# jhorstmann/queryengine

Measured on AMD Instinct MI355X. Metric: rows/sec filter+project over int64/f64 batch; achieved HBM GB/s in roofline, higher is better.
Workload: dtype int64/f64

## Files before the change

### include/qe_hip.h

```cpp
#ifndef QE_HIP_H
#define QE_HIP_H

#include <stddef.h>
#include <stdint.h>

#ifdef __cplusplus
extern "C" {
#endif

#define QE_ABI_VERSION 1

enum {
    QE_OK = 0,
    QE_ERR_INVALID_ARG = 1,
    QE_ERR_PROGRAM = 2,
    QE_ERR_HIP = 3,
    QE_ERR_OOM = 4,
    QE_ERR_UNSUPPORTED = 5,
    QE_ERR_INTERNAL = 6,
    QE_ERR_COMM = 7
};

enum {
    QE_STRING = 0,
// ... 175 lines not shown
int32_t qe_result_order_by_keys(qe_ctx *ctx, const qe_result *result, const qe_sort_key *keys, int32_t nkeys, int64_t limit,
                                qe_result **out);
int32_t qe_ctx_last_sort_stats(const qe_ctx *ctx, int64_t out[4]);

enum { QE_JOIN_INNER = 0, QE_JOIN_LEFT = 1, QE_JOIN_SEMI = 2, QE_JOIN_ANTI = 3 };
typedef struct { const qe_result *result; const qe_batch *batch; } qe_join_input;
typedef struct qe_join_table qe_join_table;

int32_t qe_join_build(qe_ctx *ctx, const qe_join_input *build, const int32_t *key_cols, int32_t nkeys,
                      qe_join_table **out);
int64_t qe_join_table_rows(const qe_join_table *table);
void    qe_join_table_free(qe_ctx *ctx, qe_join_table *table);
int32_t qe_join_probe(qe_ctx *ctx, const qe_join_table *table, const qe_join_input *probe,
                      const int32_t *key_cols, int32_t nkeys, int32_t join_type,
                      const int32_t *probe_out_cols, int32_t nprobe_out,
                      const int32_t *build_out_cols, int32_t nbuild_out, qe_result **out);
int32_t qe_ctx_last_join_stats(const qe_ctx *ctx, int64_t out[4]);

enum { QE_WIN_ROW_NUMBER = 0, QE_WIN_RANK, QE_WIN_DENSE_RANK,
       QE_WIN_SUM, QE_WIN_COUNT, QE_WIN_MIN, QE_WIN_MAX, QE_WIN_AVG,
       QE_WIN_LAG, QE_WIN_LEAD };
typedef struct { int32_t fn; int32_t column; int64_t offset; } qe_window_fn;
int32_t qe_result_window(qe_ctx *ctx, const qe_result *result,
                         const int32_t *partition_cols, int32_t npart,
                         const qe_sort_key *order, int32_t norder,
                         const qe_window_fn *fns, int32_t nfn, qe_result **out);
#define QE_FRAME_UNBOUNDED (-1)
enum { QE_WIN_FIRST_VALUE = 10, QE_WIN_LAST_VALUE = 11 };
typedef struct { int32_t fn; int32_t column; int64_t offset;
                 int64_t preceding; int64_t following; } qe_window_frame_fn;
int32_t qe_result_window_frames(qe_ctx *ctx, const qe_result *result,
                                const int32_t *partition_cols, int32_t npart,
                                const qe_sort_key *order, int32_t norder,
                                const qe_window_frame_fn *fns, int32_t nfn, qe_result **out);
int32_t qe_ctx_last_window_stats(const qe_ctx *ctx, int64_t out[4]);

enum { QE_OSA_COUNT_DISTINCT = 0, QE_OSA_PERCENTILE_CONT = 1, QE_OSA_PERCENTILE_DISC = 2, QE_OSA_MODE = 3 };
typedef struct { int32_t fn; int32_t column; double fraction; } qe_ordered_agg;
int32_t qe_result_group_ordered(qe_ctx *ctx, const qe_result *result,
                                const int32_t *group_cols, int32_t ngroup,
                                const qe_ordered_agg *fns, int32_t nfn, qe_result **out);
int32_t qe_ctx_last_ordered_stats(const qe_ctx *ctx, int64_t out[4]);

enum { QE_SET_UNION = 0, QE_SET_INTERSECT = 1, QE_SET_EXCEPT = 2 };
int32_t qe_result_set_op(qe_ctx *ctx, const qe_result *left, const qe_result *right,
                         int32_t op, int32_t all, qe_result **out);
int32_t qe_ctx_last_set_stats(const qe_ctx *ctx, int64_t out[4]);

enum { QE_ASOF_BACKWARD = 0, QE_ASOF_FORWARD = 1 };
int32_t qe_result_asof_join(qe_ctx *ctx, const qe_result *left, const qe_result *right,
                            const int32_t *left_by, const int32_t *right_by, int32_t nby,
                            int32_t left_on, int32_t right_on,
                            int32_t direction, int32_t strict, int32_t join_type,
                            const int32_t *left_out, int32_t nleft_out,
                            const int32_t *right_out, int32_t nright_out, qe_result **out);
int32_t qe_ctx_last_asof_stats(const qe_ctx *ctx, int64_t out[4]);

int32_t qe_batch_from_result(qe_ctx *ctx, const qe_result *result, qe_batch **out);

typedef struct { char internal[128]; } qe_comm_id;
int32_t qe_comm_unique_id(qe_ctx *ctx, qe_comm_id *out);
int32_t qe_comm_init(qe_ctx *ctx, int32_t nranks, int32_t rank, const qe_comm_id *id);
int32_t qe_comm_rank(const qe_ctx *ctx);
int32_t qe_comm_nranks(const qe_ctx *ctx);
void qe_comm_destroy(qe_ctx *ctx);
int32_t qe_gather(qe_ctx *ctx, const qe_result *local, int32_t root, qe_result **out);
int32_t qe_filter_project_gather(qe_ctx *ctx, const qe_batch *batch, const qe_expr *filter, const qe_expr *const *projections,
                                 int32_t nproj, int32_t root, int32_t nslices, qe_result **out);
int32_t qe_comm_allgather_host(qe_ctx *ctx, const void *send, size_t nbytes, void *recv);

int32_t qe_filter_project_source(qe_ctx *ctx, const qe_batch *batch, const qe_expr *filter,
                                 const qe_expr *const *projections, int32_t nproj, const char **out);
int32_t qe_filter_project_geometry(qe_ctx *ctx, const qe_batch *batch, const qe_expr *filter,
                                   const qe_expr *const *projections, int32_t nproj, int32_t *out_chosen,
                                   int32_t *out_from_cache);
int32_t qe_filter_project_conjunct_order(qe_ctx *ctx, const qe_batch *batch, const qe_expr *filter,
                                         const qe_expr *const *projections, int32_t nproj, int32_t *out_order, int32_t capacity,
                                         int32_t *out_nconj);
enum { QE_FORM_RING = 0, QE_FORM_TWO_PASS = 1, QE_FORM_DENSE = 2, QE_FORM_PER_NODE = 3, QE_FORM_NO_FILTER = 4,
       QE_FORM_LOCAL = 5 ,
        QE_FORM_GROUPBY_DENSE = 8, QE_FORM_GROUPBY_HASHED = 9,
       QE_FORM_GROUPBY_HASH_PARTITIONED = 10  };
int32_t qe_ctx_last_form(const qe_ctx *ctx);
int32_t qe_stream_read_bandwidth(qe_ctx *ctx, int64_t nbytes, int32_t reps, double *out_gbps);

int32_t qe_stream_read_write_time(qe_ctx *ctx, int64_t nbytes, int32_t write_every, int32_t reps, double *out_ms,
                                  double *out_written_bytes);

#ifdef __cplusplus
}
#endif
#endif
```

### queryengine_amd/csrc/qe_api.cpp

```cpp
#include <algorithm>
#include <cmath>
#include <cstdio>
#include <cstdlib>
#include <functional>
#include <sstream>

#include "qe_exec.h"
#include "qe_kernels.h"
#include "qe_pernode.h"
#include "qe_scan.h"

using namespace qe;

namespace {

constexpr double kDenseFromSelectivity = 0.12;
constexpr double kLocalUpToSelectivity = 0.03;
constexpr int64_t kSampleFromRows = 8ll << 20;

FusedGeometry geometry_of(const qe_ctx *ctx) {
    FusedGeometry g;
    const int t = ctx->opts.tuning[0], u = ctx->opts.tuning[1];
    if (t == 64 || t == 128 || t == 256 || t == 512 || t == 1024) g.threads = t;
    const int mw = ctx->opts.tuning[3] / 100;
// ... 139 lines not shown
    plan->kernel = ctx->jit->get(plan->cg.source, "qe_fused", rq.load);
    ctx->plans[k] = plan;
    return plan;
}

}

namespace {

void PlanGeometry::narrow_plan_wide_candidate() {
    if (wide && !in.dense && !agg_fns && in.group_keys.empty()) {
        size_t inbytes = 0;
        for (int c : plan->cg.used_cols) inbytes += (size_t)value_bytes(in.schema[(size_t)c].type);
        if (inbytes <= 16) {
            const FusedGeometry dflt = geometry_of(ctx);
            in.geo.subs_per_chunk = dflt.subs_per_chunk;
            in.geo.ring_entries = dflt.ring_entries;
        }
    }
}

void PlanGeometry::lds_table_1024_threads() {
    if (!in.group_keys.empty() && !plan->cg.hashed && !plan->cg.table_in_lds && ctx->opts.tuning[0] == 0 &&
        (size_t)plan->cg.ngroups * plan->cg.table_words * 8 <= 144 * 1024) {
        in.geo.threads = 1024;
        analyze();
    }
}

void PlanGeometry::hash_partitioned_tile() {
    if (plan->cg.hp && ctx->opts.tuning[1] == 0 && ctx->opts.tuning[0] == 0) {
        in.geo.threads = 512;
        int u = 4;
        auto lines_lds = [&](int uu) {
            const size_t R = (size_t)std::max(1, plan->cg.hp_line_recs), P = (size_t)plan->cg.nparts;
            const size_t tile = (size_t)(in.geo.threads / 64) * 128 * uu, lines = (tile + (P <= 256 ? 2 : 1) * (R - 1) * P + R - 1) / R;
            return lines * 132 + ((P + 3) & ~(size_t)3) * (P <= 256 ? 24 : 16) + 64;
        };
        if (plan->cg.hp_line_recs && lines_lds(4) > 156 * 1024) {
            in.hp_lines = 0;
            analyze();
        }
        if (plan->cg.hp_line_recs) {
            while (u > 1 && lines_lds(u) > 156 * 1024) u /= 2;
        } else {
            const size_t rec = (size_t)(1 + plan->cg.nvals) * 8;
            while (u > 1 && (size_t)(in.geo.threads / 64) * 128 * u * rec > 128 * 1024) u /= 2;
        }
        in.geo.unroll = u;
    }
}

void PlanGeometry::partitioned_tile_512_threads() {
    if (plan->cg.partitioned && !plan->cg.hp && plan->cg.nparts > 128 && ctx->opts.tuning[0] == 0 && in.geo.threads == 256 &&
        8 + plan->cg.part_shift + 13 <= 32 && (size_t)8 * in.geo.sub_rows() * (1 + plan->cg.nvals) * 8 <= 128 * 1024) {
        in.geo.threads = 512;
    }
}

void PlanGeometry::hashed_unroll() {
    if (plan->cg.hashed && ctx->opts.tuning[1] == 0 && in.geo.unroll > 4) {
        in.geo.unroll = 4;
    }
}

void PlanGeometry::dense_lds_tile() {
    if (in.dense) {
        const size_t rowbytes = std::max<size_t>(output_row_bytes(plan->cg.outs), 1);
        auto tile_bytes = [&]() { return (size_t)(in.geo.threads / 64) * 128 * in.geo.unroll * rowbytes; };
        const size_t limit = 64 * 1024;
        while (tile_bytes() > limit && in.geo.unroll > 1 && ctx->opts.tuning[1] == 0) in.geo.unroll /= 2;
        while (tile_bytes() > limit && in.geo.threads > 128 && ctx->opts.tuning[0] == 0) in.geo.threads /= 2;
        if (tile_bytes() > 150 * 1024)
            fail(QE_ERR_UNSUPPORTED, "projection list too wide for the dense kernel's LDS tile (" + std::to_string(rowbytes) + " bytes per output row)");
    }
}

void PlanGeometry::ring_lds_budget() {
    if (!agg_fns && in.filter && !in.dense) {
        const size_t rowbytes = std::max<size_t>(output_row_bytes(plan->cg.outs), 1);
        if (ctx->opts.tuning[7] / 100 == 0) in.geo.nbuf = 2;
        if (ctx->opts.tuning[0] == 0) {
            const size_t limit = 96 * 1024;
            while (in.geo.threads > 64 && (size_t)(in.geo.threads / 64) * in.geo.nbuf * in.geo.ring_entries * rowbytes > limit)
                in.geo.threads /= 2;
        }
        if ((size_t)(in.geo.threads / 64) * in.geo.nbuf * in.geo.ring_entries * rowbytes > 156 * 1024)
            fail(QE_ERR_UNSUPPORTED, "projection list too wide for the fused kernel's LDS buffers (" + std::to_string(rowbytes) +
                                         " bytes per output row); use QE_EXEC_PER_NODE");
    }
}

void PlanGeometry::register_estimate() {
    auto dwords = [](int t) { return (t == QE_DOUBLE || t == QE_INT64) ? 2 : 1; };
    for (;;) {
        int in_dw = 0, out_dw = 0, nbool = 1, in_nulls = 0;
        for (int c : plan->cg.used_cols) {
            in_dw += dwords(in.schema[c].type);
            in_nulls += in.schema[c].nullable ? 1 : 0;
        }
        for (const OutSpec &o : plan->cg.outs) {
            out_dw += dwords(o.type);
            nbool += o.nullable ? 1 : 0;
        }
        const int est = 2 * in.geo.unroll * (std::max(in_dw, out_dw) + nbool - 1) + (in_nulls ? in.geo.unroll : 0) + 54;
        plan->est_regs = est;
        if (((est > 168 && in.geo.unroll > 4) || (est > 300 && in.geo.unroll > 2)) && ctx->opts.tuning[1] == 0 && !wide) {
            in.geo.unroll /= 2;
            if (!in.dense) in.geo.subs_per_chunk *= 2;
            continue;
        }
        in.geo.min_waves = est <= 120 ? 4 : est <= 168 ? 3 : est <= 256 ? 2 : 1;
        break;
    }
}

void PlanGeometry::compile_without_scratch() {
    for (;;) {
        plan->cg = generate_fused_source(in);
        plan->kernel = ctx->jit->get(plan->cg.source, "qe_fused", false);
        if (ctx->jit->last_scratch <= 0) break;
        const bool can_retry = in.geo.min_waves > 1 || (in.geo.unroll > 2 && ctx->opts.tuning[1] == 0);
        if (can_retry) ctx->jit->reject(plan->cg.source, ctx->jit->last_scratch);
        if (in.geo.min_waves > 2) {
            in.geo.min_waves--;
        } else if (in.geo.unroll > 2 && ctx->opts.tuning[1] == 0) {
            in.geo.unroll /= 2;
            if (!in.dense) in.geo.subs_per_chunk *= 2;
            in.geo.min_waves = 3;
        } else if (in.geo.min_waves > 1) {
            in.geo.min_waves--;
        } else {
            break;
        }
    }
}

}

namespace qe {

int device_cus(int device) {
    int cus = 0;
    QE_HIP(hipDeviceGetAttribute(&cus, hipDeviceAttributeMultiprocessorCount, device));
    return cus > 0 ? cus : 256;
}

void fill_inputs(FusedParams &p, const qe_batch *batch, const Plan &plan) {
    std::memset(&p, 0, sizeof p);
    for (size_t s = 0; s < plan.cg.used_cols.size(); s++) {
        const Column &c = batch->cols[plan.cg.used_cols[s]];
        p.col[s] = c.data;
        p.colvalid[s] = (const unsigned long long *)c.validity;
    }
    p.nrows = batch->nrows;
    if (plan.aux_dev.size() != plan.cg.aux_tables.size()) {
        for (const std::vector<int32_t> &t : plan.cg.aux_tables) {
            void *d = nullptr;
            QE_HIP(hipMalloc(&d, std::max<size_t>(t.size() * 4, 16)));
            plan.aux_dev.push_back(d);
            if (!t.empty()) QE_HIP(hipMemcpy(d, t.data(), t.size() * 4, hipMemcpyHostToDevice));
        }
    }
    for (size_t k = 0; k < plan.aux_dev.size(); k++) p.col[kMaxCols - 1 - k] = plan.aux_dev[k];
}

void launch_fused(qe_ctx *ctx, const Plan &plan, FusedParams &p, int grid, bool timed) {
    void *args[] = {&p};
    timed = timed || ctx->opts.profile;
    if (timed) QE_HIP(hipEventRecord(ctx->ev0, ctx->stream));
    QE_HIP(hipModuleLaunchKernel(plan.kernel.fn, grid, 1, 1, plan.geo.threads, 1, 1, 0, ctx->stream, args, nullptr));
    if (timed) QE_HIP(hipEventRecord(ctx->ev1, ctx->stream));
}

void collect_time(qe_ctx *ctx) {
    if (!ctx->opts.profile) return;
    float ms = 0.f;
    QE_HIP(hipEventElapsedTime(&ms, ctx->ev0, ctx->ev1));
    ctx->last_ms = ms;
    ctx->total_ms += ms;
    ctx->launches++;
}

}

namespace {

int blocks_per_cu(const qe_ctx *ctx, const Plan &plan) {
    if (ctx->opts.tuning[3] % 100 > 0) return ctx->opts.tuning[3] % 100;
    int nb = 0;
    hipError_t e = hipModuleOccupancyMaxActiveBlocksPerMultiprocessor(&nb, plan.kernel.fn, plan.geo.threads, 0);
    if (e != hipSuccess) {
        (void)hipGetLastError();
        nb = 2;
    }
    return std::max(1, std::min(nb, 8));
}

std::vector<int> choose_conjunct_order(qe_ctx *ctx, const qe_batch *batch, const Plan &plan) {
    const int K = plan.cg.nconj;
    if (K < 2 || K > 6 || (int)plan.cg.conj_cols.size() != K) return {};
    const int64_t n = batch->nrows, sub_rows = plan.geo.sub_rows();
    const int64_t full_subs = n / sub_rows;
    const int64_t S = std::min<int64_t>(256, full_subs);
    if (S < 16) return {};
    hipFunction_t f_probe = nullptr;
    QE_HIP(hipModuleGetFunction(&f_probe, plan.kernel.module, "qe_conj_probe"));
    PoolScratch scratch(ctx);
    uint32_t *d_cnt = (uint32_t *)scratch.alloc(64 * 4);
    FusedParams pp;
    fill_inputs(pp, batch, plan);
    pp.nchunks = S;
    pp.stagger_rows = (full_subs / S) * sub_rows;
    pp.blk = (unsigned long long *)d_cnt;
    void *args[] = {&pp};
    const int waves = plan.geo.threads / 64;
    QE_HIP(hipMemsetAsync(d_cnt, 0, 64 * 4, ctx->stream));
    QE_HIP(hipModuleLaunchKernel(f_probe, (unsigned)((S + waves - 1) / waves), 1, 1, plan.geo.threads, 1, 1, 0, ctx->stream, args, nullptr));
    uint32_t h[64];
    QE_HIP(hipMemcpyAsync(h, d_cnt, sizeof h, hipMemcpyDeviceToHost, ctx->stream));
    QE_HIP(hipStreamSynchronize(ctx->stream));
    std::vector<double> rate((size_t)K);
    for (int i = 0; i < K; i++) rate[(size_t)i] = (double)h[i] / (double)(S * sub_rows);
    auto lines = [](double d, int w) { return w <= 0 ? 0.0 : (double)w * (1.0 - std::pow(1.0 - std::min(1.0, std::max(0.0, d)), 128.0 / (double)w)); };
    const size_t ncols = plan.cg.col_width.size();
    auto cost_of = [&](const std::vector<int> &perm) {
        std::vector<char> loaded(ncols, 0);
        double alive = 1.0, cost = 0.0;
        for (int k : perm) {
            for (int c : plan.cg.conj_cols[(size_t)k])
                if (!loaded[(size_t)c]) { loaded[(size_t)c] = 1; cost += lines(alive, plan.cg.col_width[(size_t)c]); }
            alive *= rate[(size_t)k];
        }
        return cost;
    };
    std::vector<int> perm((size_t)K), best;
    for (int i = 0; i < K; i++) perm[(size_t)i] = i;
    const std::vector<int> identity = perm;
    const double written = cost_of(identity);
    double best_cost = written;
    do {
        const double c = cost_of(perm);
        if (c < best_cost - 1e-9) { best_cost = c; best = perm; }
    } while (std::next_permutation(perm.begin(), perm.end()));
    if (best.empty() || best_cost > 0.97 * written) return {};
    return best;
}



template <typename Launch>
const unsigned int *with_ctrl_block(qe_ctx *ctx, Launch &&launch) {
    QE_HIP(hipMemsetAsync(ctx->d_ctrl, 0, 96, ctx->stream));
    launch();
    QE_HIP(hipMemcpyAsync(ctx->h_ctrl, ctx->d_ctrl, 96, hipMemcpyDeviceToHost, ctx->stream));
    QE_HIP(hipStreamSynchronize(ctx->stream));
    collect_time(ctx);
    return (const unsigned int *)ctx->h_ctrl;
}

unsigned long long *alloc_trace(qe_ctx *ctx, PoolScratch &scratch, int64_t nchunks) {
    if (!debug_bit(ctx, kDbgTrace)) return nullptr;
    void *trace = scratch.alloc((size_t)nchunks * 32);
    QE_HIP(hipMemsetAsync(trace, 0, (size_t)nchunks * 32, ctx->stream));
    return (unsigned long long *)trace;
}

void dump_trace_file(const unsigned long long *d_trace, int64_t nchunks) {
    const char *path = d_trace ? std::getenv("QE_TRACE_FILE") : nullptr;
    if (!path) return;
    std::vector<unsigned long long> tr((size_t)nchunks * 4);
    QE_HIP(hipMemcpy(tr.data(), d_trace, tr.size() * 8, hipMemcpyDeviceToHost));
    if (FILE *f = std::fopen(path, "wb")) {
        std::fwrite(tr.data(), 8, tr.size(), f);
        std::fclose(f);
    }
}

struct FusedRun {
    qe_ctx *ctx;
    const qe_batch *batch;
    const Plan &plan;
    FusedParams p;
    qe_result *res;
    int64_t cap;
};

void alloc_staging(const FusedRun &r, PoolScratch &scratch, FusedParams &p, size_t rows) {
    for (size_t i = 0; i < r.res->cols.size(); i++) {
        const OutColumn &oc = r.res->cols[i];
        const size_t w = oc.type == QE_BOOLEAN ? 1 : type_width(oc.type);
        p.stage[i] = scratch.alloc(rows * w);
        if (oc.nullable) p.stagevalid[i] = (unsigned char *)scratch.alloc(rows);
    }
}

struct GeoPick {
    qe_ctx::GeoChoice *choice = nullptr;
    int cand = 0;
    std::shared_ptr<Plan> plan;
    bool exploring() const { return choice && choice->chosen < 0; }
};

GeoPick pick_geometry_candidate(qe_ctx *ctx, const qe_batch *batch, const PlanRequest &ordered, const std::shared_ptr<Plan> &obase) {
    GeoPick pick;
    pick.plan = obase;
    const int64_t n = batch->nrows;
    const int k2 = obase->geo.unroll > 0 ? (obase->est_regs - 54) / (2 * obase->geo.unroll) : 99;
    const bool eligible = !obase->explicit_geometry && obase->est_regs > 0 && n >= (32ll << 20) &&
                          32 * k2 + 54 <= 256 && !debug_bit(ctx, kDbgNoGeometryChoice);
    if (!eligible) return pick;
    const bool fresh = ctx->geo_choice.find(obase.get()) == ctx->geo_choice.end();
    qe_ctx::GeoChoice *choice = pick.choice = &ctx->geo_choice[obase.get()];
    if (fresh) {
        double margin = 1.0;
        const int saved = ctx->jit->load_choice(obase->cg.source, &margin);
        if (saved >= 0 && margin >= 0.07) { choice->chosen = saved; choice->from_cache = true; }
    }
    int cand = choice->chosen;
    if (cand < 0) {
        cand = 0;
        for (int c = 1; c < qe_ctx::GeoChoice::kCands; c++)
            if (choice->runs[c] < choice->runs[cand]) cand = c;
    }
    if (cand >= 1) {
        try {
            PlanRequest rq = ordered;
            rq.geo_cand = cand;
            pick.plan = get_plan(ctx, batch, rq);
        } catch (const Error &) {
            choice->runs[cand] = 1 << 20;
            if (choice->chosen == cand) choice->chosen = 0;
            cand = 0;
            pick.plan = obase;
        }
    }
    pick.cand = cand;
    return pick;
// ... 150 lines not shown
    dp.desc = desc;
    dp.l1 = desc + nchunks;
    dp.blk = desc + nchunks + nblocks;
    dp.ticket = ctx->d_ctrl;
    dp.error = ctx->d_ctrl + 1;
    dp.total = (unsigned long long *)(ctx->d_ctrl + 2);
    dp.nchunks = nchunks;
    dp.trace = alloc_trace(ctx, trace_scratch, nchunks);
    const unsigned int *hc = with_ctrl_block(ctx, [&] {
        QE_HIP(hipMemsetAsync(desc, 0, desc_words * 8, ctx->stream));
        launch_fused(ctx, dplan, dp, grid);
    });
    dump_trace_file(dp.trace, nchunks);
    if (hc[1] != 0)
        fail(QE_ERR_INTERNAL, hc[1] == 2 ? "dense kernel: ticket grant never posted (spin limit)"
                                         : "dense kernel: look-back spin limit reached (chunk descriptor never published)");
    return (int64_t)ctx->h_ctrl[1];
}

int64_t run_two_pass(const FusedRun &r) {
    qe_ctx *ctx = r.ctx;
    const Plan &plan = r.plan;
    const int64_t n = r.batch->nrows;
    const int64_t chunk_rows = plan.geo.chunk_rows();
    const int waves = plan.geo.threads / 64;
    const int64_t nchunks = (n + chunk_rows - 1) / chunk_rows;
    const int grid = (int)std::max<int64_t>(1, std::min<int64_t>((nchunks + waves - 1) / waves, (int64_t)device_cus(ctx->device) * 8));
    hipFunction_t f_count = nullptr, f_write = nullptr;
    QE_HIP(hipModuleGetFunction(&f_count, plan.kernel.module, "qe_fp_count"));
    QE_HIP(hipModuleGetFunction(&f_write, plan.kernel.module, "qe_fp_write"));
    PoolScratch scratch(ctx);
    uint32_t *d_counts = (uint32_t *)scratch.alloc((size_t)nchunks * 4);
    FusedParams p = r.p;
    p.capacity = r.cap;
    p.nchunks = nchunks;
    p.blk = (unsigned long long *)d_counts;
    p.error = ctx->d_ctrl + 1;
    p.total = (unsigned long long *)(ctx->d_ctrl + 2);
    void *args[] = {&p};
    with_ctrl_block(ctx, [&] {
        if (ctx->opts.profile) QE_HIP(hipEventRecord(ctx->ev0, ctx->stream));
        QE_HIP(hipModuleLaunchKernel(f_count, grid, 1, 1, plan.geo.threads, 1, 1, 0, ctx->stream, args, nullptr));
        launch_carry_scan<uint32_t, 256>(ctx->stream, d_counts, nchunks, 1, p.total);
        QE_HIP(hipModuleLaunchKernel(f_write, grid, 1, 1, plan.geo.threads, 1, 1, 0, ctx->stream, args, nullptr));
        if (ctx->opts.profile) QE_HIP(hipEventRecord(ctx->ev1, ctx->stream));
    });
    return (int64_t)ctx->h_ctrl[1];
}

struct RingChunks {
    int64_t nchunks = 0, stagger_chunks = 0, stagger_rows = 0;
};
RingChunks ring_chunks(int64_t n, int64_t chunk_rows, int64_t stagger_chunks) {
    RingChunks rc;
    const int64_t sixteenth = chunk_rows / 16;
    const int64_t periods = std::min<int64_t>(stagger_chunks / 16, n / (136 * sixteenth));
    int64_t c = periods * 16, rows = periods * 136 * sixteenth;
    while (c < stagger_chunks && rows < n) {
        rows += (((7 * c) & 15) + 1) * sixteenth;
        c++;
    }
    rc.stagger_rows = rows;
    if (rows >= n) {
        rc.nchunks = rc.stagger_chunks = c;
    } else {
        rc.stagger_chunks = stagger_chunks;
        rc.nchunks = stagger_chunks + (n - rows + chunk_rows - 1) / chunk_rows;
    }
    return rc;
}

int64_t run_ring(const FusedRun &r, const GeoPick &pick, const Plan &obase) {
    qe_ctx *ctx = r.ctx;
    const Plan &plan = r.plan;
    const int64_t n = r.batch->nrows;
    const int64_t chunk_rows = plan.geo.chunk_rows();
    const int waves = plan.geo.threads / 64;
    const int64_t max_grid = (int64_t)device_cus(ctx->device) * blocks_per_cu(ctx, plan);
    const RingChunks rc = ring_chunks(n, chunk_rows, plan.geo.stagger ? max_grid * waves : 0);
    const int64_t nchunks = rc.nchunks;
    if (nchunks >= (1ll << 31)) fail(QE_ERR_UNSUPPORTED, "batch too large for 32-bit chunk tickets");
    const int grid = (int)std::min<int64_t>((nchunks + waves - 1) / waves, max_grid);
    static const bool dbg_grid = std::getenv("QE_DEBUG_GRID") != nullptr;
    if (dbg_grid) std::fprintf(stderr, "[qe] ring kernel: grid %d x %d threads (%d blocks per CU), unroll %d, %d sub-tiles per chunk, ring %d, min_waves %d\n",
                               grid, plan.geo.threads, blocks_per_cu(ctx, plan), plan.geo.unroll, plan.geo.subs_per_chunk, plan.geo.ring_entries, plan.geo.min_waves);
    PoolScratch scratch(ctx);
    const int64_t nblocks = (nchunks + 63) / 64;
    const size_t desc_words = (size_t)nchunks + 2 * (size_t)nblocks;
    unsigned long long *desc = (unsigned long long *)scratch.alloc(desc_words * 8);
    FusedParams p = r.p;
    if (plan.cg.has_filter) {
        const size_t slots = (size_t)grid * waves * plan.geo.nbuf;
        alloc_staging(r, scratch, p, slots * (size_t)plan.geo.slot_rows());
    }
    p.capacity = r.cap;
    p.desc = desc;
    p.l1 = desc + nchunks;
    p.blk = desc + nchunks + nblocks;
    p.ticket = ctx->d_ctrl;
    p.error = ctx->d_ctrl + 1;
    p.total = (unsigned long long *)(ctx->d_ctrl + 2);
    p.nchunks = nchunks;
    p.stagger_chunks = rc.stagger_chunks;
    p.stagger_rows = rc.stagger_rows;
    p.stats = (unsigned long long *)(ctx->d_ctrl + 16);
    p.trace = alloc_trace(ctx, scratch, nchunks);
    const unsigned int *hc = with_ctrl_block(ctx, [&] {
        QE_HIP(hipMemsetAsync(desc, 0, desc_words * 8, ctx->stream));
        launch_fused(ctx, plan, p, grid, pick.exploring());
    });
    if (pick.exploring()) record_geometry_timing(ctx, pick, obase, n);
    dump_trace_file(p.trace, nchunks);
    if (debug_bit(ctx, kDbgWaitStats))
        std::fprintf(stderr, "[qe stats] chunks %llu failed_tries %llu forced_waits %llu blocking_spins %llu\n", ctx->h_ctrl[11],
                     ctx->h_ctrl[8], ctx->h_ctrl[10], ctx->h_ctrl[9]);
    if (hc[1] != 0) fail(QE_ERR_INTERNAL, "fused kernel: look-back spin limit reached (tile descriptor never published)");
    return (int64_t)ctx->h_ctrl[1];
}

void alloc_outputs(qe_ctx *ctx, const Plan &plan, qe_result *res, int64_t cap, FusedParams &p) {
    for (size_t i = 0; i < res->cols.size(); i++) {
        OutColumn &oc = res->cols[i];
        if (oc.type == QE_BOOLEAN) {
            oc.bytes_data = ctx->pool.alloc((size_t)cap);
            p.out[i] = oc.bytes_data;
        } else {
            oc.data = ctx->pool.alloc(type_width(oc.type) * (size_t)cap);
            p.out[i] = oc.data;
        }
        if (oc.nullable) {
            oc.bytes_valid = (uint8_t *)ctx->pool.alloc((size_t)cap);
            p.outvalid[i] = oc.bytes_valid;
        }
    }
}

void pack_byte_columns(qe_ctx *ctx, qe_result *res) {
    bool packed = false;
    for (OutColumn &oc : res->cols) {
        if (oc.type == QE_BOOLEAN) {
            oc.data = ctx->pool.alloc(bitmap_bytes(res->count));
            launch_pack_bytes(ctx->stream, (const uint8_t *)oc.bytes_data, res->count, (uint64_t *)oc.data);
            packed = true;
        }
        if (oc.nullable) {
            oc.validity = (uint64_t *)ctx->pool.alloc(bitmap_bytes(res->count));
            launch_pack_bytes(ctx->stream, oc.bytes_valid, res->count, oc.validity);
            packed = true;
        }
    }
    if (!packed) return;
    QE_HIP(hipGetLastError());
    QE_HIP(hipStreamSynchronize(ctx->stream));
    for (OutColumn &oc : res->cols) {
        ctx->pool.release(oc.bytes_data);
        ctx->pool.release(oc.bytes_valid);
        oc.bytes_data = nullptr;
        oc.bytes_valid = nullptr;
    }
}

qe_result *run_fused(qe_ctx *ctx, const qe_batch *batch, const qe_expr *filter, const qe_expr *const *projs,
                     int32_t nproj) {
    const PlanRequest written{filter, projs, nproj};
    const std::shared_ptr<Plan> base = get_plan(ctx, batch, written);
    const int64_t n = batch->nrows;
    if (base->cg.has_probe && !base->conj_decided && n >= kSampleFromRows && !debug_bit(ctx, kDbgWrittenConjunctOrder)) {
        base->conj_decided = true;
        base->conj_order = choose_conjunct_order(ctx, batch, *base);
    }
    const std::vector<int> order = base->conj_order;
    PlanRequest ordered = written;
    if (!order.empty()) ordered.conj_order = &order;
    const std::shared_ptr<Plan> obase = order.empty() ? base : get_plan(ctx, batch, ordered);
    const GeoPick pick = pick_geometry_candidate(ctx, batch, ordered, obase);
    const Plan &plan = *pick.plan;

    ResultPtr res = new_result(ctx, 0);
    const int64_t cap = ctx->opts.result_capacity_rows > 0 ? std::min<int64_t>(ctx->opts.result_capacity_rows, n) : n;
    res->capacity = cap;
    for (const OutSpec &os : plan.cg.outs) {
        OutColumn oc;
        oc.type = os.type;
        oc.nullable = os.nullable;
        oc.dict = os.dict;
        oc.dict_handle.d = os.dict;
        res->cols.push_back(oc);
    }
    if (n == 0) return res.release();
    FusedRun run{ctx, batch, plan, {}, res.get(), cap};
    fill_inputs(run.p, batch, plan);
    alloc_outputs(ctx, plan, res.get(), cap, run.p);

    const FormSwitches sw = form_switches(ctx);
    if (plan.cg.has_filter && plan.cg.two_pass && base->last_selectivity < 0 && !sw.force_dense && !sw.never_dense && !sw.force_two_pass &&
        n >= kSampleFromRows && !debug_bit(ctx, kDbgNoSelectivitySample))
        base->last_selectivity = sample_selectivity(run);
    Form form = choose_form(plan.cg, base->last_selectivity, base->local_overflowed, n, sw);
    int64_t total = 0;
// ... 179 lines not shown
```

### queryengine_amd/csrc/qe_codegen.cpp

```cpp
#include "qe_expr_rules.h"

#include <algorithm>
#include <cinttypes>
#include <cmath>
#include <cstdio>
#include <sstream>

namespace qe {

namespace {

const char *kPrelude1 = R"QE(
// ---- generated by libqe_hip: fused filter+project kernel for gfx950 ----
typedef unsigned long long u64;
typedef long long i64;
typedef unsigned int u32;
typedef double  qe_f64x2 __attribute__((ext_vector_type(2)));
typedef i64     qe_i64x2 __attribute__((ext_vector_type(2)));
typedef int     qe_i32x2 __attribute__((ext_vector_type(2)));
typedef u64     u64x2 __attribute__((ext_vector_type(2)));
// Bitmap words (validity, BOOLEAN values) are wave-uniform: read through the constant address space they become SCALAR loads
// (s_load_dwordx4 into SGPRs).  As plain global loads hipcc issued one 16-byte VECTOR load per group and bitmap in which all 64
// lanes fetch the same two words into four VGPRs each -- 48 VGPRs per sub-tile for three nullable columns.  The batch is
// read-only while a kernel runs and the scalar cache starts every kernel invalidated.
// ... 1451 lines not shown
                                *(u64x2 *)(ln + idx * QE_GB_NV + v) = rv;
                            }
                        } else {
#pragma unroll
                            for (int v = 0; v < QE_GB_NV; ++v) ln[idx * QE_GB_NV + v] = sv.val[v][u][r];
                        }
                        ((u32 *)(ln + QE_GB_META))[idx] = (u32)(tile0 + (i64)(wave * QE_SUB_ROWS + u * 128 + 2 * lane + r));
                        if (QE_GB_FLAGS) ((unsigned char *)(ln + QE_GB_META) + 4u * QE_GB_PADU)[idx] = (unsigned char)(w & 255u);
                        if (idx == 0u) L.lineglob[line] = pos / QE_GB_PADU;   // (a run fills its lines from slot 0 on)
                        continue;
                    }
#endif
                    const u64 h = ((u64)pos << 32) | ((u64)(u32)(wave * QE_SUB_ROWS + u * 128 + 2 * lane + r) << (8 + QE_GB_SHIFT)) | ((u64)((w >> 9) & (QE_GB_GP - 1u)) << 8) | (u64)(w & 255u);
                    if (QE_GB_RECW % 2 == 0) {
                        u64x2 rv;
                        rv.x = h;
                        rv.y = sv.val[0][u][r];
                        *(u64x2 *)(L.stage + (size_t)slot * QE_GB_RECW) = rv;
#pragma unroll
                        for (int w = 2; w < QE_GB_RECW; w += 2) {   // record word w (>= 1) is value w - 1
                            u64x2 r2;
                            r2.x = sv.val[w - 1][u][r];
                            r2.y = sv.val[w][u][r];
                            *(u64x2 *)(L.stage + (size_t)slot * QE_GB_RECW + w) = r2;
                        }
                    } else {
                        L.stage[(size_t)slot * QE_GB_RECW] = h;
#pragma unroll
                        for (int v = 0; v < QE_GB_NV; ++v) L.stage[(size_t)slot * QE_GB_RECW + 1 + v] = sv.val[v][u][r];
                    }
                }
            }
        }
    }
}
)QE";
}

void Emitter::access_macros() {
    s << (in.nontemporal ? "#define QE_LD(p) __builtin_nontemporal_load(p)\n" : "#define QE_LD(p) (*(p))\n");
    s << (in.nt_stores ? "#define QE_ST(p, v) __builtin_nontemporal_store((v), (p))\n" : "#define QE_ST(p, v) (*(p) = (v))\n");
    s << (in.nt_stores == 2 ? "#define QE_SPILL_ST(p, v) __builtin_nontemporal_store((v), (p))\n" : "#define QE_SPILL_ST(p, v) (*(p) = (v))\n");
    s << "#define QE_VEC_ST " << (in.vec_stores ? 1 : 0) << "\n";
}

void Emitter::row_functions() {
    for (size_t ci = 0; ci < a.conj_body.size(); ci++) {
        s << "\n__device__ __forceinline__ void qe_conj" << ci << "(const QeParams &p, ";
        for (int j = 0; j < NC; j++) {
            const BoundColumn &bc = col(j);
            s << "const " << ctype(bc.type) << " c" << j << ", ";
            if (bc.nullable) s << "const bool kc" << j << ", ";
        }
        s << "bool &alive) {\n    (void)p;\n";
        for (int j = 0; j < NC; j++) {
            s << "    (void)c" << j << ";";
            if (col(j).nullable) s << " (void)kc" << j << ";";
        }
        s << "\n" << a.conj_body[ci] << "}\n";
    }
    s << "\n__device__ __forceinline__ void qe_row(const QeParams &p";
    bool first = false;
    for (int j = 0; j < NC; j++) {
        const BoundColumn &bc = col(j);
        s << (first ? "" : ", ") << "const " << ctype(bc.type) << " c" << j;
        first = false;
        if (bc.nullable) s << ", const bool kc" << j;
    }
    s << (first ? "" : ", ") << "bool &keep";
    for (int i = 0; i < NO; i++) {
        s << ", " << ctype(out.outs[i].type) << " &o" << i;
        if (out.outs[i].nullable) s << ", bool &ok" << i;
    }
    if (a.row_grp()) s << ", int &grp";
    if (a.row_keys()) {
        for (size_t i = 0; i < in.group_keys.size(); i++) s << ", u64 &kw" << i;
        s << ", u32 &knull";
    }
    s << ") {\n    (void)p;\n" << a.row_body << "}\n";
}

void Emitter::ring_defs() {
    const FusedGeometry &geo = in.geo;
    s << "\n#define QE_NBUF " << geo.nbuf << "u\n#define QE_RING " << geo.ring_entries << "   // LDS entries per wave, buffer and output column (power of two)\n";
    s << "#define QE_FL_RING " << out.fl_ring << "\n";
    s << "struct QeRing {\n";
    for (int i = 0; i < NO; i++) {
        const OutSpec &os = out.outs[i];
        s << "    " << (os.type == QE_BOOLEAN ? "unsigned char" : ctype(os.type)) << " *r" << i << ";\n";
        if (os.nullable) s << "    unsigned char *rv" << i << ";\n";
    }
    if (NO == 0) s << "    int unused;\n";
    s << "};\n";
}

std::string Emitter::valid_arg(int j) const { return "((qe_vb[u] >> (" + std::to_string(a.vbit[j]) + " + r)) & 1u) != 0u"; }

void Emitter::loads(int stage, bool guarded) {
    s << "#pragma unroll\n    for (int u = 0; u < QE_U; ++u) {\n";
    s << "        const i64 r0 = sub0 + u * 128 + 2 * lane;\n";
    s << "        const i64 g0 = (sub0 + u * 128) >> 6;   // wave-uniform bitmap word index (even)\n";
    s << "        const u32 sh = (u32)(2 * lane) & 63u;\n";
    s << "        const i64 nwords = (p.nrows + 63) >> 6;\n        (void)nwords; (void)g0; (void)sh; (void)r0;\n";
    if (guarded) s << "        if (keep[u][0] || keep[u][1]) {\n";
    for (int j = 0; j < NC; j++) {
        if (stage >= 0 && a.col_stage[j] != stage) continue;
        const BoundColumn &bc = col(j);
        auto bitmap_load = [&](const std::string &ptr, const std::string &dst, int vb = -1) {
            s << "        {\n            const qe_cu64p bm = (qe_cu64p)(u64)(" << ptr << ");\n";
            s << "            u64 w0, w1;\n";
            s << "            if (FULL) { w0 = bm[g0]; w1 = bm[g0 + 1]; }\n";
            s << "            else { w0 = g0 < nwords ? bm[g0] : 0ull; w1 = g0 + 1 < nwords ? bm[g0 + 1] : 0ull; }\n";
            s << "            const u64 w = lane < 32 ? w0 : w1;\n";
            if (vb >= 0) {
                s << "            qe_vb[u] |= ((u32)(w >> sh) & 3u) << " << vb << ";\n        }\n";
            } else {
                s << "            " << dst << "[u][0] = (w >> sh) & 1ull;\n";
                s << "            " << dst << "[u][1] = (w >> (sh + 1u)) & 1ull;\n        }\n";
            }
        };
        if (a.vonly[(size_t)j]) {
            const std::string ct = bc.type == QE_BOOLEAN ? "bool" : ctype(bc.type);
            s << "        c" << j << "[u][0] = (" << ct << ")0; c" << j << "[u][1] = (" << ct << ")0;\n";
        } else if (bc.type == QE_BOOLEAN) {
            bitmap_load("(const u64 *)p.col[" + std::to_string(j) + "]", "c" + std::to_string(j));
        } else {
            const std::string ct = ctype(bc.type), vt = load_vec_type(bc.type);
            s << "        {\n            const " << ct << " *src = (const " << ct << " *)p.col[" << j << "] + r0;\n";
            s << "            if (FULL) { const " << vt << " v = QE_LD((const " << vt << " *)src); c" << j
              << "[u][0] = v.x; c" << j << "[u][1] = v.y; }\n";
            s << "            else { c" << j << "[u][0] = r0 < p.nrows ? src[0] : (" << ct << ")0; c" << j
              << "[u][1] = r0 + 1 < p.nrows ? src[1] : (" << ct << ")0; }\n        }\n";
        }
        if (bc.nullable) bitmap_load("p.colvalid[" + std::to_string(j) + "]", "", a.vbit[j]);
    }
    if (guarded) s << "        }\n";
    s << "    }\n";
}

void Emitter::prefetch_loader() {
    bool s0_nulls = false;
    s << "\nstruct QeS0 {\n";
    for (int j = 0; j < NC; j++) {
        if (a.col_stage[j] != 0) continue;
        const BoundColumn &bc = col(j);
        s << "    " << (bc.type == QE_BOOLEAN ? "bool" : ctype(bc.type)) << " c" << j << "[QE_U][2];\n";
        s0_nulls = s0_nulls || bc.nullable;
    }
    if (s0_nulls) s << "    u32 vb[QE_U];\n";
    s << "};\n// issue the stage-0 loads of the (full) sub-tile at sub0\n"
         "__device__ __forceinline__ void qe_s0_load(const QeParams &p, const i64 sub0, const int lane, QeS0 &s0) {\n"
         "    constexpr bool FULL = true;\n";
    for (int j = 0; j < NC; j++)
        if (a.col_stage[j] == 0) s << "    auto &c" << j << " = s0.c" << j << ";\n";
    if (s0_nulls) s << "    auto &qe_vb = s0.vb;\n#pragma unroll\n    for (int u = 0; u < QE_U; ++u) qe_vb[u] = 0u;\n";
    loads(0, false);
    s << "}\n";
}

std::string Emitter::col_args() const {
    std::string args;
    for (int j = 0; j < NC; j++) {
        args += (args.empty() ? "" : ", ") + std::string("c") + std::to_string(j) + "[u][r]";
        if (col(j).nullable) args += ", " + valid_arg(j);
    }
    return args;
}

void Emitter::row_call(bool only_alive) {
// ... 205 lines not shown
        s << indent << "if (rowid < " << ld("e") << ") QE_GB_MIN_U64(e, rowid);   // monotone: a stale (larger) value only costs an atomic\n";
        for (int i = 0; i < NO; i++) {
            const int fn = in.agg_fns[i];
            std::string cond = out.outs[i].nullable ? "ok" + std::to_string(i) + "[u][r]" : "true";
            std::string val = "(double)o" + std::to_string(i) + "[u][r]";
            const std::string cntp = "e + " + std::to_string(1 + 2 * i), accp = "(i64 *)(e + " + std::to_string(2 + 2 * i) + ")";
            s << indent << "if (" << cond << ") { ";
            if (out.cnt_src[i] == i) {
                if (acc_real_count[(size_t)i]) s << "QE_GB_ADD_U64(" << cntp << ", 1ull); ";
                else s << "if (" << ld(cntp) << " == 0ull) __hip_atomic_store(" << cntp << ", 1ull, __ATOMIC_RELAXED, " << scope << "); ";
            }
            if (fn == QE_AGG_SUM || fn == QE_AGG_AVG) s << "QE_GB_ADD_F64((double *)(e + " << 2 + 2 * i << "), " << val << "); ";
            else if (fn == QE_AGG_MIN) s << "{ const i64 kv = qe_ord_key(" << val << ", true); if (kv < " << ld(accp) << ") QE_GB_MIN_I64(" << accp << ", kv); } ";
            else if (fn == QE_AGG_MAX) s << "{ const i64 kv = qe_ord_key(" << val << ", false); if (kv > " << ld(accp) << ") QE_GB_MAX_I64(" << accp << ", kv); } ";
            s << "}\n";
        }
    };
    s << "                u64 key[QE_HT_NK];\n";
    for (size_t i = 0; i < in.group_keys.size(); i++) s << "                key[" << i << "] = kw" << i << "[u][r];\n";
    s << "                const u64 kn = (u64)knull[u][r];\n";
    s << "                u64 *slot = qe_ht_find<false>(tab, QE_HT_LDS - 1u, qe_ht_hash_lds(key, kn), key, kn, 32, (u32 *)nullptr);\n";
    s << "                if (slot != nullptr) {\n                    u64 *e = slot + QE_HT_ACC;\n";
    emit_accumulate("                    ", false);
    s << "                } else {\n";
    s << "                    if (p.stagger_chunks != 0) { *p.error = 4u; continue; }   // the keys do not fit LDS: the host resolves them to dense ids instead (qe_ht_build)\n";
    s << "                    slot = qe_ht_find<true>(gtab, (u32)p.capacity - 1u, qe_ht_hash(key, kn), key, kn, 4096, p.ticket);\n";
    s << "                    if (slot == nullptr) { *p.error = 3u; continue; }   // table too small: the host grows it and runs again\n";
    s << "                    u64 *e = slot + QE_HT_ACC;\n";
    emit_accumulate("                    ", true);
    s << "                }\n";
    s << "            }\n        }\n    }\n}\n";
}

void Emitter::table_accumulate() {
    s << "                u64 *e = tab + (i64)grp[u][r] * " << out.table_words << ";\n";
    s << "                if (rowid < __hip_atomic_load(e, __ATOMIC_RELAXED, __HIP_MEMORY_SCOPE_WORKGROUP)) QE_GB_MIN_U64(e, rowid);   // monotone: a stale (larger) value only costs an atomic\n";
    const std::string dscope = out.table_in_lds ? "__HIP_MEMORY_SCOPE_WORKGROUP" : "__HIP_MEMORY_SCOPE_AGENT";
    for (int i = 0; i < NO; i++) {
        const int fn = in.agg_fns[i];
        std::string cond = out.outs[i].nullable ? "ok" + std::to_string(i) + "[u][r]" : "true";
        std::string val = "(double)o" + std::to_string(i) + "[u][r]";
        const std::string accp = "(i64 *)(e + " + std::to_string(2 + 2 * i) + ")";
        s << "                if (" << cond << ") { ";
        if (out.cnt_src[i] == i) s << "QE_GB_ADD_U64(e + " << 1 + 2 * i << ", 1ull); ";
        if (fn == QE_AGG_SUM || fn == QE_AGG_AVG) s << "QE_GB_ADD_F64((double *)(e + " << 2 + 2 * i << "), " << val << "); ";
        else if (fn == QE_AGG_MIN) s << "{ const i64 kv = qe_ord_key(" << val << ", true); if (kv < __hip_atomic_load(" << accp << ", __ATOMIC_RELAXED, " << dscope << ")) QE_GB_MIN_I64(" << accp << ", kv); } ";
        else if (fn == QE_AGG_MAX) s << "{ const i64 kv = qe_ord_key(" << val << ", false); if (kv > __hip_atomic_load(" << accp << ", __ATOMIC_RELAXED, " << dscope << ")) QE_GB_MAX_I64(" << accp << ", kv); } ";
        s << "}\n";
    }
    s << "            }\n        }\n    }\n}\n";
}

void Emitter::compaction_tail() {
    s << R"QE(    if (MODE == 1) {   // two-pass form, pass 1: kept rows of the chunk
#pragma unroll
        for (int u = 0; u < QE_U; ++u) run += (u32)__popcll(__ballot(keep[u][0])) + (u32)__popcll(__ballot(keep[u][1]));
        return;
    }
    if (MODE == 2) {   // two-pass form, pass 2: rows are ordered (u, lane, r); stage_base = position of the chunk's first kept row
#pragma unroll
        for (int u = 0; u < QE_U; ++u) {
            const u64 b0 = __ballot(keep[u][0]);
            const u64 b1 = __ballot(keep[u][1]);
            const u32 off = run + qe_mbcnt(b0) + qe_mbcnt(b1);
            run += (u32)__popcll(b0) + (u32)__popcll(b1);
#pragma unroll
            for (int r = 0; r < 2; ++r) {
                const u64 pos = stage_base + off + (r == 1 && keep[u][0] ? 1u : 0u);
                if (keep[u][r] && (i64)pos < p.capacity) {
)QE";
    for (int i = 0; i < NO; i++) {
        const OutSpec &os = out.outs[i];
        const std::string ct = os.type == QE_BOOLEAN ? "unsigned char" : ctype(os.type);
        if (os.type == QE_BOOLEAN) s << "                    ((unsigned char *)p.out[" << i << "])[pos] = (unsigned char)(o" << i << "[u][r] ? 1 : 0);\n";
        else s << "                    ((" << ct << " *)p.out[" << i << "])[pos] = o" << i << "[u][r];\n";
        if (os.nullable) s << "                    p.outvalid[" << i << "][pos] = (unsigned char)(ok" << i << "[u][r] ? 1 : 0);\n";
    }
    s << R"QE(                }
            }
        }
        return;
    }
    // rows are ordered (u, lane, r) inside the sub-tile: lane offsets from ballots; the ring belongs to this wave only
#pragma unroll
    for (int u = 0; u < QE_U; ++u) {
        const u64 b0 = __ballot(keep[u][0]);
        const u64 b1 = __ballot(keep[u][1]);
        const u32 off = run + qe_mbcnt(b0) + qe_mbcnt(b1);
        run += (u32)__popcll(b0) + (u32)__popcll(b1);
#pragma unroll
        for (int r = 0; r < 2; ++r) {
            if (keep[u][r] && (QE_DEBUG_MASK & 2)) {   // ablation build: keep the outputs (and their loads) alive
)QE";
    for (int i = 0; i < NO; i++) s << "                asm volatile(\"\" :: \"v\"(o" << i << "[u][r]));\n";
    s << R"QE(            }
            if (keep[u][r] && !(QE_DEBUG_MASK & 2)) {
                const u32 slot = (off + (r == 1 && keep[u][0] ? 1u : 0u)) & ((MODE == 3 ? QE_FL_RING : QE_RING) - 1);
)QE";
    for (int i = 0; i < NO; i++) {
        const OutSpec &os = out.outs[i];
        if (os.type == QE_BOOLEAN) s << "                ring.r" << i << "[slot] = o" << i << "[u][r] ? 1 : 0;\n";
        else s << "                ring.r" << i << "[slot] = o" << i << "[u][r];\n";
        if (os.nullable) s << "                ring.rv" << i << "[slot] = ok" << i << "[u][r] ? 1 : 0;\n";
    }
    s << "            }\n        }\n";
    s << "        while (MODE != 3 && run - flushed >= QE_RING - 128u) {   // only when the ring would overflow (high selectivity); the local form (MODE 3) flags the overflow at the end of its chunk instead\n";
    s << "            const u32 src = (flushed + lane) & (QE_RING - 1);\n";
    s << "            const u64 dst = stage_base + flushed + lane;\n            if (!(QE_DEBUG_MASK & 8)) {\n";
    for (int i = 0; i < NO; i++) {
        const OutSpec &os = out.outs[i];
        const std::string ct = os.type == QE_BOOLEAN ? "unsigned char" : ctype(os.type);
        s << "            QE_SPILL_ST((" << ct << " *)p.stage[" << i << "] + dst, ring.r" << i << "[src]);\n";
        if (os.nullable) s << "            QE_SPILL_ST(p.stagevalid[" << i << "] + dst, ring.rv" << i << "[src]);\n";
    }
    s << "            }\n            flushed += 64u;\n        }\n    }\n}\n";
}

void Emitter::passthrough_tail() {
    s << "    (void)stage_base; (void)run; (void)flushed; (void)ring;\n";
    s << "#pragma unroll\n    for (int u = 0; u < QE_U; ++u) {\n#pragma unroll\n        for (int r = 0; r < 2; ++r) {\n";
    s << "            const i64 idx = sub0 + u * 128 + 2 * lane + r;\n";
    s << "            if (keep[u][r] && idx < p.capacity) {\n";
    for (int i = 0; i < NO; i++) {
        const OutSpec &os = out.outs[i];
        if (os.type == QE_BOOLEAN) s << "                ((unsigned char *)p.out[" << i << "])[idx] = o" << i << "[u][r] ? 1 : 0;\n";
        else s << "                ((" << ctype(os.type) << " *)p.out[" << i << "])[idx] = o" << i << "[u][r];\n";
        if (os.nullable) s << "                p.outvalid[" << i << "][idx] = ok" << i << "[u][r] ? 1 : 0;\n";
    }
    s << "            }\n        }\n    }\n}\n";
}

void Emitter::conj_probe() {
    s << "\nextern \"C\" __global__ void __launch_bounds__(QE_THREADS) qe_conj_probe(const QeParams p) {\n"
         "    const int lane = threadIdx.x & 63;\n    constexpr bool FULL = true;\n"
         "    const i64 wslot = (i64)blockIdx.x * QE_WAVES + (threadIdx.x >> 6), nslots = (i64)gridDim.x * QE_WAVES;\n";
    for (size_t ci = 0; ci < a.conj_body.size(); ci++) s << "    u32 cnt" << ci << " = 0;\n";
    s << "    for (i64 sidx = wslot; sidx < p.nchunks; sidx += nslots) {\n        const i64 sub0 = sidx * p.stagger_rows;\n";
    for (int j = 0; j < NC; j++) {
        const BoundColumn &bc = col(j);
        s << "        " << (bc.type == QE_BOOLEAN ? "bool" : ctype(bc.type)) << " c" << j << "[QE_U][2];\n";
    }
    {
        bool anynull = false;
        for (int j = 0; j < NC; j++) anynull = anynull || a.vbit[j] >= 0;
        if (anynull) s << "        u32 qe_vb[QE_U] = {};\n";
    }
    for (int st = 0; st < (int)a.conj_body.size(); st++) {
        bool any = false;
        for (int j = 0; j < NC; j++) any = any || a.col_stage[j] == st;
        if (any) loads(st, false);
    }
    s << "#pragma unroll\n        for (int u = 0; u < QE_U; ++u) {\n#pragma unroll\n            for (int r = 0; r < 2; ++r) {\n                bool alive;\n";
    {
        std::string args;
        for (int j = 0; j < NC; j++) {
            const BoundColumn &bc = col(j);
            const bool loaded = a.col_stage[j] < (int)a.conj_body.size();
            args += (args.empty() ? "" : ", ") + (loaded ? std::string("c") + std::to_string(j) + "[u][r]" : std::string("(") + (bc.type == QE_BOOLEAN ? "bool" : ctype(bc.type)) + ")0");
            if (bc.nullable) args += loaded ? ", " + valid_arg(j) : ", false";
        }
        for (size_t ci = 0; ci < a.conj_body.size(); ci++)
            s << "                qe_conj" << ci << "(p, " << args << (args.empty() ? "" : ", ") << "alive);\n                cnt" << ci
              << " += (u32)__popcll(__ballot(alive));\n";
    }
    s << "            }\n        }\n    }\n";
    for (size_t ci = 0; ci < a.conj_body.size(); ci++) s << "    if (lane == 0 && cnt" << ci << ") atomicAdd((u32 *)p.blk + " << ci << ", cnt" << ci << ");\n";
    s << "}\n";
}

void Emitter::filter_project_head() {
    header();
    access_macros();
    row_functions();
    ring_defs();
    if (a.prefetch) prefetch_loader();
    s << "#define QE_PREFETCH " << (a.prefetch ? 1 : 0) << "\ntypedef " << (a.prefetch ? "QeS0" : "int") << " QePf;\n";
    sub_head("\n// MODE 0: compaction into the wave's LDS ring (single pass); 1: count the kept rows only; 2: store every kept row at\n"
     "// stage_base + its rank inside the chunk (two-pass form: the chunk's offset is already known); 3: as 0 but the ring is never\n"
     "// spilled (local form: a chunk that keeps more rows than the ring holds is reported, the host runs another form)\n"
     "// PF: the stage-0 columns arrive in `pf` (loaded by the previous call / the prologue); the stage-0 loads of the sub-tile at\n"
     "// next_sub0 (a FULL one; -1: none) are issued into it\n"
     "template <bool FULL, int MODE, bool PF, typename Hook>\n__device__ __forceinline__ void qe_sub(const QeParams &p, const i64 sub0, const int lane, Hook &&after_loads",
             ", const QeRing &ring, const u64 stage_base, u32 &run, u32 &flushed, QePf &pf, const i64 next_sub0", true, false);
    if (a.has_filter) compaction_tail();
    else passthrough_tail();
}

void Emitter::dense() {
    filter_project_head();
    s << "\nstruct QeIn {\n";
    for (int j = 0; j < NC; j++) {
        const BoundColumn &bc = col(j);
        s << "    " << (bc.type == QE_BOOLEAN ? "bool" : ctype(bc.type)) << " c" << j << "[QE_U][2];\n";
    }
    bool dense_nulls = false;
    for (int j = 0; j < NC; j++) dense_nulls = dense_nulls || a.vbit[j] >= 0;
    if (dense_nulls) s << "    u32 vb[QE_U];\n";
    if (NC == 0) s << "    int unused;\n";
// ... 142 lines not shown
            if ((QE_DEBUG_MASK & 32) && lane == 0) p.trace[tile * 4 + 1] = __builtin_amdgcn_s_memrealtime();
            u32 t_next = 0;
            if (lane == 0) t_next = atomicAdd(p.ticket, 1u);   // the next tile: its round trip runs under the look-back below
            qe_publish_complete(p, tile, tile_total, old, lane);
            if (parked) {                  // resolve the tile parked one iteration ago: its predecessors have had a whole tile's time
                QeLb lb;
                qe_lb_init(lb, ptile);
                const u64 excl = qe_lookback_wait(p, ptile, lb, lane);
                if (lane == 0 && ptile > 0)
                    __hip_atomic_store(p.desc + ptile, QE_ST_PREFIX | (excl + pcount), __ATOMIC_RELAXED, __HIP_MEMORY_SCOPE_AGENT);
                if (lane == 0 && (ptile & 63) == 63)
                    __hip_atomic_fetch_max(p.l1 + (ptile >> 6), QE_ST_PREFIX | (excl + pcount), __ATOMIC_RELAXED, __HIP_MEMORY_SCOPE_AGENT);
                if (lane == 0) s_excl = excl;
                if ((QE_DEBUG_MASK & 32) && lane == 0) p.trace[ptile * 4 + 2] = __builtin_amdgcn_s_memrealtime();
            }
            if (lane == 0) s_ticket[par ^ 1u] = t_next;
        }
        __syncthreads();                   // (B) the next ticket and the parked tile's offset are known
        const i64 next = (i64)__hip_atomic_load(&s_ticket[par ^ 1u], __ATOMIC_RELAXED, __HIP_MEMORY_SCOPE_WORKGROUP);
        if ((QE_DEBUG_MASK & 32) && threadIdx.x == 0 && next < p.nchunks) p.trace[next * 4 + 0] = __builtin_amdgcn_s_memrealtime();
        if (next < p.nchunks) {            // the inputs are dead: the next tile's loads go out before anything else
            const i64 nsub = (next * QE_WAVES + wv) * (i64)QE_SUB_ROWS;
            if (nsub + QE_SUB_ROWS <= p.nrows) qe_dense_load<true>(p, nsub, lane, in);
            else qe_dense_load<false>(p, nsub, lane, in);
        }
        if (parked) {
            qe_dense_move(p, tl, pcount, s_excl);
            if ((QE_DEBUG_MASK & 32) && threadIdx.x == 0) p.trace[ptile * 4 + 3] = __builtin_amdgcn_s_memrealtime();
            __syncthreads();               // (C) the LDS tile is free again
        }
        qe_dense_park(lane, out, tl, wave_off);
        parked = true;
        ptile = tile;
        pcount = tile_total;
        if (next >= p.nchunks) break;      // tile ids only grow: nothing is left for this workgroup (uniform)
        tile = next;
    }
    // drain: the last parked tile
    __syncthreads();
    if (wv == 0) {
        QeLb lb;
        qe_lb_init(lb, ptile);
        const u64 excl = qe_lookback_wait(p, ptile, lb, lane);
        if (lane == 0 && ptile > 0)
            __hip_atomic_store(p.desc + ptile, QE_ST_PREFIX | (excl + pcount), __ATOMIC_RELAXED, __HIP_MEMORY_SCOPE_AGENT);
        if (lane == 0 && ((ptile & 63) == 63 || ptile == p.nchunks - 1))
            __hip_atomic_fetch_max(p.l1 + (ptile >> 6), QE_ST_PREFIX | (excl + pcount), __ATOMIC_RELAXED, __HIP_MEMORY_SCOPE_AGENT);
        if (lane == 0 && ptile == p.nchunks - 1) *p.total = excl + pcount;
        if (lane == 0) s_excl = excl;
        if ((QE_DEBUG_MASK & 32) && lane == 0) p.trace[ptile * 4 + 2] = __builtin_amdgcn_s_memrealtime();
    }
    __syncthreads();
    qe_dense_move(p, tl, pcount, s_excl);
    if ((QE_DEBUG_MASK & 32) && threadIdx.x == 0) p.trace[ptile * 4 + 3] = __builtin_amdgcn_s_memrealtime();
}
)QE";
}

void Emitter::ring_kernel() {
    const bool has_filter = a.has_filter;
    s << R"QE(
// Rows of chunk c.  The first p.stagger_chunks chunks have graded sizes ((7c mod 16)+1)/16 of a full
// chunk so that the waves, which all start together, do not finish (and look back) in lockstep.
__device__ __forceinline__ i64 qe_stagger_prefix(i64 c) {   // sub-tiles before staggered chunk c
    const i64 unit = QE_CHUNK_ROWS / QE_SUB_ROWS / 16;      // sub-tiles per 1/16 chunk
    i64 sixteenths = (c >> 4) * 136;                        // a full period of 16 sums to 1+2+...+16
    for (i64 k = c & ~15ll; k < c; ++k) sixteenths += ((7 * k) & 15) + 1;
    return sixteenths * unit;
}
__device__ __forceinline__ void qe_chunk_range(const QeParams &p, const i64 c, i64 &row0, i64 &rend) {
    if (c < p.stagger_chunks) {
        row0 = qe_stagger_prefix(c) * QE_SUB_ROWS;
        rend = row0 + ((((7 * c) & 15) + 1) * (i64)(QE_CHUNK_ROWS / 16));
    } else {
        row0 = p.stagger_rows + (c - p.stagger_chunks) * (i64)QE_CHUNK_ROWS;
        rend = row0 + QE_CHUNK_ROWS;
    }
    rend = rend < p.nrows ? rend : p.nrows;
}

)QE";
    if (has_filter) {
        s << R"QE(
// The exclusive prefix of a streamed chunk is known: tell the successors at once.
__device__ __forceinline__ void qe_publish_prefix(const QeParams &p, const i64 pchunk, const u32 prun, const u64 excl, const int lane) {
    if (lane == 0 && pchunk > 0)
        __hip_atomic_store(p.desc + pchunk, QE_ST_PREFIX | (excl + prun), __ATOMIC_RELAXED, __HIP_MEMORY_SCOPE_AGENT);
    if (lane == 0 && ((pchunk & 63) == 63 || pchunk == p.nchunks - 1))   // last chunk of its block: the block's inclusive prefix
        __hip_atomic_fetch_max(p.l1 + (pchunk >> 6), QE_ST_PREFIX | (excl + prun), __ATOMIC_RELAXED, __HIP_MEMORY_SCOPE_AGENT);
    if (lane == 0 && pchunk == p.nchunks - 1) *p.total = excl + prun;
}
// Output-write gate: with QE_GATE_PERIOD != 0 the rows of a resolved chunk are moved only while a device-wide window
// of the shared 100 MHz clock is open, so that the (expensive) trickle of writes reaches the memory system in bursts.
__device__ __forceinline__ bool qe_gate_open() {
    if (QE_GATE_PERIOD == 0) return true;
    return ((u32)__builtin_amdgcn_s_memrealtime() & (u32)(QE_GATE_PERIOD - 1)) < (u32)QE_GATE_WIDTH;
}
// Finish a streamed chunk whose exclusive prefix is known: publish the inclusive prefix, then move the
// staged rows to their final, globally ordered position (coalesced both ways, 4 blocks in flight).
// Rows [0, pflushed) of the chunk were spilled to the wave's staging slot (only when the LDS buffer
// overflowed); rows [pflushed, prun) are still in the LDS buffer `ring`.
__device__ __forceinline__ void qe_finish(const QeParams &p, const i64 pchunk, const u32 prun, const u32 pflushed, const u64 pbase,
                                          const u64 excl, const int lane, const QeRing &ring, const bool publish = true) {
    if (publish) qe_publish_prefix(p, pchunk, prun, excl, lane);
    if ((QE_DEBUG_MASK & 32) && lane == 0) p.trace[pchunk * 4 + 2] = __builtin_amdgcn_s_memrealtime();
    if (!(QE_DEBUG_MASK & 4)) {
        // LDS-resident part: straight from the buffer to its final position
#if QE_VEC_ST
        // two rows per lane: 8-byte columns leave in 16-byte stores (1 KiB per wave instruction, half the store instructions);
        // one row is peeled off when the chunk's first position is odd, so that every pair starts on a 16-byte boundary
        u32 jv = pflushed;
        if (((excl + jv) & 1ull) != 0 && jv < prun) {
            const u64 pos = excl + jv;
            if (lane == 0 && (i64)pos < p.capacity) {
)QE";
        for (int i = 0; i < NO; i++) {
            const OutSpec &os = out.outs[i];
            const std::string ct = os.type == QE_BOOLEAN ? "unsigned char" : ctype(os.type);
            s << "                QE_ST((" << ct << " *)p.out[" << i << "] + pos, ring.r" << i << "[jv & (QE_RING - 1)]);\n";
            if (os.nullable) s << "                QE_ST(p.outvalid[" << i << "] + pos, ring.rv" << i << "[jv & (QE_RING - 1)]);\n";
        }
        s << R"QE(            }
            jv++;
        }
        for (u32 j = jv + 2u * lane; j < prun; j += 128u) {
            const u64 pos = excl + j;
            const bool two = j + 1u < prun && (i64)(pos + 1) < p.capacity;
            if ((i64)pos < p.capacity) {
)QE";
        for (int i = 0; i < NO; i++) {
            const OutSpec &os = out.outs[i];
            const std::string ct = os.type == QE_BOOLEAN ? "unsigned char" : ctype(os.type);
            const std::string a = "ring.r" + std::to_string(i) + "[j & (QE_RING - 1)]", b = "ring.r" + std::to_string(i) + "[(j + 1u) & (QE_RING - 1)]";
            if (os.type == QE_DOUBLE || os.type == QE_INT64) {
                const std::string vt = os.type == QE_DOUBLE ? "qe_f64x2" : "qe_i64x2";
                s << "                if (two) { " << vt << " v2; v2.x = " << a << "; v2.y = " << b << "; QE_ST((" << vt << " *)((" << ct << " *)p.out[" << i
                  << "] + pos), v2); }\n                else QE_ST((" << ct << " *)p.out[" << i << "] + pos, " << a << ");\n";
            } else {
                s << "                QE_ST((" << ct << " *)p.out[" << i << "] + pos, " << a << ");\n                if (two) QE_ST((" << ct << " *)p.out[" << i
                  << "] + pos + 1, " << b << ");\n";
            }
            if (os.nullable)
                s << "                QE_ST(p.outvalid[" << i << "] + pos, ring.rv" << i << "[j & (QE_RING - 1)]);\n                if (two) QE_ST(p.outvalid[" << i
                  << "] + pos + 1, ring.rv" << i << "[(j + 1u) & (QE_RING - 1)]);\n";
        }
        s << R"QE(            }
        }
#else
        for (u32 j = pflushed + lane; j < prun; j += 64u) {
            const u64 pos = excl + j;
            if ((i64)pos < p.capacity) {
)QE";
        for (int i = 0; i < NO; i++) {
            const OutSpec &os = out.outs[i];
            const std::string ct = os.type == QE_BOOLEAN ? "unsigned char" : ctype(os.type);
            s << "                QE_ST((" << ct << " *)p.out[" << i << "] + pos, ring.r" << i << "[j & (QE_RING - 1)]);\n";
            if (os.nullable) s << "                QE_ST(p.outvalid[" << i << "] + pos, ring.rv" << i << "[j & (QE_RING - 1)]);\n";
        }
        s << R"QE(            }
        }
#endif
    }
    if (pflushed == 0) return;
    asm volatile("s_waitcnt vmcnt(0)" ::: "memory");   // this wave's own staging stores have landed
    const u32 mrun = (QE_DEBUG_MASK & 4) ? 0u : pflushed;
    for (u32 j0 = 0; j0 < mrun; j0 += 256u) {
)QE";
        for (int i = 0; i < NO; i++) {
            const OutSpec &os = out.outs[i];
            const std::string ct = os.type == QE_BOOLEAN ? "unsigned char" : ctype(os.type);
            s << "        " << ct << " m" << i << "[4];\n";
            if (os.nullable) s << "        unsigned char mv" << i << "[4];\n";
        }
        s << "#pragma unroll\n        for (int q = 0; q < 4; ++q) {\n            const u32 j = j0 + q * 64 + lane;\n";
        s << "            if (j < mrun) {\n";
        for (int i = 0; i < NO; i++) {
            const OutSpec &os = out.outs[i];
            const std::string ct = os.type == QE_BOOLEAN ? "unsigned char" : ctype(os.type);
            s << "                m" << i << "[q] = ((const " << ct << " *)p.stage[" << i << "])[pbase + j];\n";
            if (os.nullable) s << "                mv" << i << "[q] = p.stagevalid[" << i << "][pbase + j];\n";
        }
        s << "            }\n        }\n";
        s << "#pragma unroll\n        for (int q = 0; q < 4; ++q) {\n            const u32 j = j0 + q * 64 + lane;\n";
        s << "            const u64 pos = excl + j;\n            if (j < mrun && (i64)pos < p.capacity) {\n";
        for (int i = 0; i < NO; i++) {
            const OutSpec &os = out.outs[i];
            const std::string ct = os.type == QE_BOOLEAN ? "unsigned char" : ctype(os.type);
            s << "                QE_ST((" << ct << " *)p.out[" << i << "] + pos, m" << i << "[q]);\n";
            if (os.nullable) s << "                QE_ST(p.outvalid[" << i << "] + pos, mv" << i << "[q]);\n";
        }
        s << "            }\n        }\n    }\n}\n";
    }
    s << R"QE(
// Every WAVE is an independent worker: it draws a chunk of consecutive rows with one ticket, streams it
// sub-tile by sub-tile and (with a Filter) compacts the kept rows into one of its QE_NBUF private LDS
// buffers, then publishes the chunk's count.  Chunk ids are monotone in start order, so a look-back only
// ever waits on chunks that are already running.  Streamed chunks queue up in the wave's FIFO of LDS
// buffers; the OLDEST one is resolved (look-back + move) NON-BLOCKINGLY at sub-tile boundaries while the
// wave keeps streaming newer chunks; the wave waits only when every buffer is taken.  At low selectivity
// the rows never leave LDS before they are written to their final position.  No barrier.
extern "C" __global__ void __launch_bounds__(QE_THREADS, QE_MIN_WAVES) qe_fused(const QeParams p) {
    const int lane = threadIdx.x & 63;
    const int wv = __builtin_amdgcn_readfirstlane(threadIdx.x >> 6);
    const u32 wslot = __builtin_amdgcn_readfirstlane(blockIdx.x * QE_WAVES + (threadIdx.x >> 6));
    QeRing ring, pring;
)QE";
    if (has_filter) {
        for (int i = 0; i < NO; i++) {
            const OutSpec &os = out.outs[i];
            const std::string ct = os.type == QE_BOOLEAN ? "unsigned char" : ctype(os.type);
            s << "    __shared__ " << ct << " s_r" << i << "[QE_WAVES][QE_NBUF * QE_RING];\n";
            if (os.nullable) s << "    __shared__ unsigned char s_rv" << i << "[QE_WAVES][QE_NBUF * QE_RING];\n";
        }
        s << "    __shared__ u32 s_meta[QE_WAVES][QE_NBUF][4];   // per queued chunk: id, kept rows, rows spilled to staging\n";
    } else {
        for (int i = 0; i < NO; i++) {
            s << "    ring.r" << i << " = nullptr; pring.r" << i << " = nullptr;\n";
            if (out.outs[i].nullable) s << "    ring.rv" << i << " = nullptr; pring.rv" << i << " = nullptr;\n";
        }
    }
    s << R"QE(    (void)wv;
    u32 cur = 0;                 // LDS buffer being filled
    u32 npend = 0;               // streamed chunks queued in buffers cur-npend .. cur-1 (mod QE_NBUF), oldest first
    i64 hchunk = 0;              // the oldest queued chunk (head of the FIFO) ...
    u32 hrun = 0, hflushed = 0;  // ... its kept rows and how many of them were spilled to its staging slot
    bool hvalid = false;         // head fields + look-back state are loaded
    bool hres = false;           // the head's exclusive prefix is known (published), its rows are not moved yet
    u64 hexcl = 0;
    QeLb lb;                     // resumable look-back state of the head
    qe_lb_init(lb, 0);
    u64 st_fail = 0, st_spin = 0, st_forced = 0, st_chunks = 0;
    u32 nsub_done = 0, nchunk_done = 0;
    bool pub_owed = false;       // a block-counter add whose return value has not been looked at yet
    i64 pub_chunk = 0;
    u32 pub_run = 0;
    u64 pub_old = 0;
    u32 t_next = 0;              // ticket drawn during the last sub-tile of the previous chunk
    bool t_have = false;
)QE";
    if (has_filter) {
        s << R"QE(    auto load_head = [&]() {
        const u32 h = (cur + QE_NBUF - npend) % QE_NBUF;
        hchunk = (i64)s_meta[wv][h][0];
        hrun = s_meta[wv][h][1];
        hflushed = s_meta[wv][h][2];
        qe_lb_init(lb, hchunk);
        hvalid = true;
)QE";
        for (int i = 0; i < NO; i++) {
            s << "        pring.r" << i << " = s_r" << i << "[wv] + h * QE_RING;\n";
            if (out.outs[i].nullable) s << "        pring.rv" << i << " = s_rv" << i << "[wv] + h * QE_RING;\n";
        }
        s << R"QE(    };
    auto head_base = [&]() { return ((u64)wslot * QE_NBUF + (cur + QE_NBUF - npend) % QE_NBUF) * QE_SLOT_ROWS; };
)QE";
    }
    s << R"QE(    for (;;) {
        // The ticket is drawn at most ONE sub-tile before the wave starts the chunk: a ticket held for a whole
        u32 t = t_next;
        if (QE_DEBUG_MASK & 64) {   // ablation build: static strided chunks instead of tickets (no progress guarantee)
            t = wslot + nchunk_done * (gridDim.x * QE_WAVES);
            t_have = true;
        }
        if (!t_have && lane == 0) t = atomicAdd(p.ticket, 1u);
        t_have = false;
        const i64 chunk = (i64)(u32)__builtin_amdgcn_readfirstlane(t);
        const bool have = chunk < p.nchunks;
        if ((QE_DEBUG_MASK & 32) && have && lane == 0) p.trace[chunk * 4 + 0] = __builtin_amdgcn_s_memrealtime();
        const u64 stage_base = ((u64)wslot * QE_NBUF + cur) * QE_SLOT_ROWS;
        u32 run = 0, flushed = 0;
)QE";
    if (has_filter) {
        for (int i = 0; i < NO; i++) {
            s << "        ring.r" << i << " = s_r" << i << "[wv] + cur * QE_RING;\n";
            if (out.outs[i].nullable) s << "        ring.rv" << i << " = s_rv" << i << "[wv] + cur * QE_RING;\n";
        }
    }
    s << R"QE(        if (have) {
            i64 row0, rend;
            qe_chunk_range(p, chunk, row0, rend);
            i64 sub = row0;
            u32 si = 0;
            // issued right after each sub-tile's loads, so that its stores / polls run under them
            auto hook = [&]() {
)QE";
    if (has_filter)
        s << "                if (pub_owed) { qe_publish_complete(p, pub_chunk, pub_run, pub_old, lane); pub_owed = false; }\n";
    if (has_filter)
        s << "                if (npend > 0 && (si >= QE_RESOLVE_AT || npend > 1)) {   // non-blocking: try the oldest, else keep streaming\n"
             "                    if (!hvalid) load_head();\n"
             "                    if (!hres) {\n"
             "                        u64 excl;\n"
             "                        if ((QE_DEBUG_MASK & 1) || qe_lookback_step(p, hchunk, lb, lane, excl)) {\n"
             "                            hres = true; hexcl = (QE_DEBUG_MASK & 1) ? 0ull : excl;\n"
             "                            qe_publish_prefix(p, hchunk, hrun, hexcl, lane);\n"
             "                        } else if (QE_DEBUG_MASK & 16) st_fail++;\n"
             "                    }\n"
             "                    // resolved: move the rows now, or (gated build) in the next window / before the buffer is needed\n"
             "                    if (hres && (si + 2 >= QE_SUBS_PER_CHUNK || qe_gate_open())) {\n"
             "                        qe_finish(p, hchunk, hrun, hflushed, head_base(), hexcl, lane, pring, false);\n"
             "                        npend--; hvalid = false; hres = false;\n                    }\n                }\n";
    s << R"QE(            };
            if (QE_PRIO_MODE == 2) qe_rotate_priority(nchunk_done);
            QePf pf;
#if QE_PREFETCH
            if (sub + QE_SUB_ROWS <= rend) qe_s0_load(p, sub, lane, pf);   // the chunk's first sub-tile; every later one is prefetched by its predecessor
#endif
            for (; sub + QE_SUB_ROWS <= rend; sub += QE_SUB_ROWS, ++si) {
                if (QE_PRIO_MODE == 1 || QE_PRIO_MODE == 3) qe_rotate_priority(nsub_done++);
                if (sub + 2 * QE_SUB_ROWS > rend && !t_have && !(QE_DEBUG_MASK & 64)) {   // last full sub-tile: draw the next ticket now
                    if (lane == 0) t_next = atomicAdd(p.ticket, 1u);
                    t_have = true;
                }
                qe_sub<true, 0, QE_PREFETCH != 0>(p, sub, lane, hook, ring, stage_base, run, flushed, pf,
                                                  sub + 2 * QE_SUB_ROWS <= rend ? sub + QE_SUB_ROWS : (i64)-1);
            }
            nchunk_done++;
            if (sub < rend) qe_sub<false, 0, false>(p, sub, lane, hook, ring, stage_base, run, flushed, pf, (i64)-1);
)QE";
    if (has_filter) {
        s << R"QE(            // publish this chunk's count at once (chunk 0 knows its prefix already) and queue it
            if (!(QE_DEBUG_MASK & 128)) {   // (ablation bit 128: no descriptor traffic at all)
                if (pub_owed) qe_publish_complete(p, pub_chunk, pub_run, pub_old, lane);
                pub_old = qe_publish_issue(p, chunk, run, lane);
                pub_owed = true; pub_chunk = chunk; pub_run = run;
            }
            if ((QE_DEBUG_MASK & 32) && lane == 0) {
                p.trace[chunk * 4 + 1] = __builtin_amdgcn_s_memrealtime();
                p.trace[chunk * 4 + 3] = ((u64)wslot << 40) | ((u64)(__builtin_amdgcn_s_getreg((20 << 0) | (0 << 6) | (3 << 11)) & 0xf) << 32) |
                                         (u64)(u32)__builtin_amdgcn_s_getreg((4 << 0) | (0 << 6) | (31 << 11));
            }
            if (lane == 0) { s_meta[wv][cur][0] = (u32)chunk; s_meta[wv][cur][1] = run; s_meta[wv][cur][2] = flushed; }
            npend++;
            cur = (cur + 1u) % QE_NBUF;
            st_chunks++;
        }
        if (pub_owed && (npend == QE_NBUF || !have)) { qe_publish_complete(p, pub_chunk, pub_run, pub_old, lane); pub_owed = false; }
        // every buffer is taken (or nothing is left to stream): now the wave may wait for the oldest chunk
        while (npend == QE_NBUF || (!have && npend > 0)) {
            if (!hvalid) load_head();
            if (QE_DEBUG_MASK & 16) {
                st_forced++;
                u64 e2;
                QeLb l2 = lb;
                while (!qe_lookback_step(p, hchunk, l2, lane, e2)) { st_spin++; __builtin_amdgcn_s_sleep(32); if (st_spin > (1ull << 24)) break; }
            }
            const u64 excl = hres ? hexcl : ((QE_DEBUG_MASK & 1) ? 0ull : qe_lookback_wait(p, hchunk, lb, lane));
            qe_finish(p, hchunk, hrun, hflushed, head_base(), excl, lane, pring, !hres);
            npend--; hvalid = false; hres = false;
        }
        if (!have) break;
)QE";
    } else {
        s << "            if (lane == 0 && chunk == p.nchunks - 1) *p.total = (u64)p.nrows;\n        }\n";
        s << "        (void)npend; (void)hchunk; (void)hrun; (void)hflushed; (void)hvalid; (void)hres; (void)hexcl; (void)cur; (void)pring; (void)run; (void)flushed; (void)lb;\n";
        s << "        if (!have) break;\n";
    }
    s << "    }\n";
    if (has_filter)
        s << "    if ((QE_DEBUG_MASK & 16) && lane == 0) { atomicAdd(p.stats + 0, st_fail); atomicAdd(p.stats + 1, st_spin); "
             "atomicAdd(p.stats + 2, st_forced); atomicAdd(p.stats + 3, st_chunks); }\n";
    s << "    (void)st_fail; (void)st_spin; (void)st_forced; (void)st_chunks; (void)nsub_done; (void)nchunk_done; (void)pub_owed; (void)pub_chunk; (void)pub_run; (void)pub_old; (void)t_next; (void)t_have;\n}\n";
}

void Emitter::two_pass_and_local() {
    s << R"QE(
// ---- two-pass form (high selectivity): every wave owns whole chunks (static stride) in BOTH passes ----
// pass 1: kept rows per chunk -> ((u32 *)p.blk)[chunk]
extern "C" __global__ void __launch_bounds__(QE_THREADS) qe_fp_count(const QeParams p) {
    const int lane = threadIdx.x & 63;
    const i64 wslot = (i64)blockIdx.x * QE_WAVES + (threadIdx.x >> 6), nslots = (i64)gridDim.x * QE_WAVES;
    QeRing ring = {};
    QePf pf;
    // p.stagger_chunks > 1: a SAMPLE -- every stagger_chunks-th chunk only (the first execution of a plan estimates its
    // selectivity from 256 chunks spread over the batch and picks the ring or the dense form from that)
    const i64 every = p.stagger_chunks > 1 ? p.stagger_chunks : 1;
    for (i64 c = __builtin_amdgcn_readfirstlane((int)wslot); c < p.nchunks; c += nslots) {
        const i64 row0 = c * every * QE_CHUNK_ROWS;
        const i64 rend = row0 + QE_CHUNK_ROWS < p.nrows ? row0 + QE_CHUNK_ROWS : p.nrows;
        u32 run = 0, flushed = 0;
        for (i64 sub = row0; sub < rend; sub += QE_SUB_ROWS) {
            if (sub + QE_SUB_ROWS <= p.nrows) qe_sub<true, 1, false>(p, sub, lane, []() {}, ring, 0ull, run, flushed, pf, (i64)-1);
            else qe_sub<false, 1, false>(p, sub, lane, []() {}, ring, 0ull, run, flushed, pf, (i64)-1);
        }
        if (lane == 0) ((u32 *)p.blk)[c] = run;
    }
}
// pass 2: ((u32 *)p.blk)[chunk] is now the position of the chunk's first kept row (exclusive scan): evaluate again and
// store every kept row at its final place, in input order
extern "C" __global__ void __launch_bounds__(QE_THREADS) qe_fp_write(const QeParams p) {
    const int lane = threadIdx.x & 63;
    const i64 wslot = (i64)blockIdx.x * QE_WAVES + (threadIdx.x >> 6), nslots = (i64)gridDim.x * QE_WAVES;
    QeRing ring = {};
    QePf pf;
    for (i64 c = __builtin_amdgcn_readfirstlane((int)wslot); c < p.nchunks; c += nslots) {
        const i64 row0 = c * QE_CHUNK_ROWS;
        const i64 rend = row0 + QE_CHUNK_ROWS < p.nrows ? row0 + QE_CHUNK_ROWS : p.nrows;
        const u64 base = (u64)((const u32 *)p.blk)[c];
        u32 run = 0, flushed = 0;
        for (i64 sub = row0; sub < rend; sub += QE_SUB_ROWS) {
            if (sub + QE_SUB_ROWS <= p.nrows) qe_sub<true, 2, false>(p, sub, lane, []() {}, ring, base, run, flushed, pf, (i64)-1);
            else qe_sub<false, 2, false>(p, sub, lane, []() {}, ring, base, run, flushed, pf, (i64)-1);
        }
    }
}

// ---- LOCAL form (plans that keep a few per cent of their rows at most) -------------------------------------------------
// The scan has NO inter-wave dependency at all: every wave owns whole chunks of p.stagger_rows rows (static stride), compacts
// a chunk's kept rows in its LDS ring exactly as the single-pass kernel does and then parks them, in row order, in the
// chunk's own slot of QE_FL_RING rows in a staging area (p.stage) next to the chunk's count (((u32 *)p.blk)[chunk]).  No ticket
// (one ticket address serves ~80 chunks / us: a plan that streams 4-byte codes hits that limit), no descriptor, no
// look-back.  A scan over the counts and qe_fl_move (below) then put the rows at their final place: the kept rows are written
// twice and read once more, which is nothing at the selectivities this form is chosen for (the host sizes the chunk so that
// it keeps about QE_FL_RING / 4 rows).  A chunk that keeps more rows than its slot holds is reported through p.error (5): the
// host runs the single-pass kernel instead and remembers that for the plan.
extern "C" __global__ void __launch_bounds__(QE_THREADS) qe_fl_scan(const QeParams p) {   // (no occupancy request: it must never spill)
    const int lane = threadIdx.x & 63;
    const int wv = __builtin_amdgcn_readfirstlane(threadIdx.x >> 6);
    const i64 wslot = (i64)blockIdx.x * QE_WAVES + wv, nslots = (i64)gridDim.x * QE_WAVES;
    QeRing ring;
)QE";
    for (int i = 0; i < NO; i++) {
        const OutSpec &os = out.outs[i];
        const std::string ct = os.type == QE_BOOLEAN ? "unsigned char" : ctype(os.type);
        s << "    __shared__ " << ct << " s_l" << i << "[QE_WAVES][QE_FL_RING];\n    ring.r" << i << " = s_l" << i << "[wv];\n";
        if (os.nullable) s << "    __shared__ unsigned char s_lv" << i << "[QE_WAVES][QE_FL_RING];\n    ring.rv" << i << " = s_lv" << i << "[wv];\n";
    }
    if (NO == 0) s << "    ring.unused = 0;\n";
    s << R"QE(    u32 nsub_done = 0;
    QePf pf;
    bool pf_have = false;   // `pf` holds the stage-0 columns of the next full sub-tile this wave works on (also across its chunks)
    (void)pf_have;
    for (i64 c = __builtin_amdgcn_readfirstlane((int)wslot); c < p.nchunks; c += nslots) {
        const i64 row0 = c * p.stagger_rows;
        const i64 rend = row0 + p.stagger_rows < p.nrows ? row0 + p.stagger_rows : p.nrows;
        u32 run = 0, flushed = 0;
        for (i64 sub = row0; sub < rend; sub += QE_SUB_ROWS) {
            if (QE_PRIO_MODE != 0) qe_rotate_priority(nsub_done++);
            if (sub + QE_SUB_ROWS <= p.nrows) {
#if QE_PREFETCH
                i64 nx = sub + QE_SUB_ROWS < rend ? sub + QE_SUB_ROWS : (c + nslots < p.nchunks ? (c + nslots) * p.stagger_rows : (i64)-1);
                if (nx >= 0 && nx + QE_SUB_ROWS > p.nrows) nx = -1;   // only full sub-tiles are prefetched
                if (!pf_have) qe_s0_load(p, sub, lane, pf);
                qe_sub<true, 3, true>(p, sub, lane, []() {}, ring, 0ull, run, flushed, pf, nx);
                pf_have = nx >= 0;
#else
                qe_sub<true, 3, false>(p, sub, lane, []() {}, ring, 0ull, run, flushed, pf, (i64)-1);
#endif
            } else {
                qe_sub<false, 3, false>(p, sub, lane, []() {}, ring, 0ull, run, flushed, pf, (i64)-1);
            }
        }
        const u32 m = run < (u32)QE_FL_RING ? run : (u32)QE_FL_RING;
        const u64 base = (u64)c * QE_FL_RING;
        for (u32 j = lane; j < m; j += 64u) {
)QE";
    for (int i = 0; i < NO; i++) {
        const OutSpec &os = out.outs[i];
        const std::string ct = os.type == QE_BOOLEAN ? "unsigned char" : ctype(os.type);
        s << "            ((" << ct << " *)p.stage[" << i << "])[base + j] = ring.r" << i << "[j];\n";
        if (os.nullable) s << "            p.stagevalid[" << i << "][base + j] = ring.rv" << i << "[j];\n";
    }
    s << R"QE(        }
        if (lane == 0) {
            ((u32 *)p.blk)[c] = run;
            if (run > (u32)QE_FL_RING) *p.error = 5u;
        }
    }
    (void)nsub_done;
}
// the chunks' exclusive offsets are in ((const u32 *)p.l1): one wave per chunk moves its rows from the slot to their final,
// globally ordered position (input order: chunks in order, rows of a chunk in rank order)
extern "C" __global__ void __launch_bounds__(256) qe_fl_move(const QeParams p) {
    const int lane = threadIdx.x & 63;
    const i64 wslot = (i64)blockIdx.x * 4 + (threadIdx.x >> 6), nslots = (i64)gridDim.x * 4;
    const u32 *counts = (const u32 *)p.blk, *offsets = (const u32 *)p.l1;
    for (i64 c = __builtin_amdgcn_readfirstlane((int)wslot); c < p.nchunks; c += nslots) {
        const u32 n = counts[c] < (u32)QE_FL_RING ? counts[c] : (u32)QE_FL_RING;   // (an overflowed chunk: the host discards this execution's rows, but nothing may be read past the slot)
        const u64 off = (u64)offsets[c], base = (u64)c * QE_FL_RING;
        for (u32 j = lane; j < n; j += 64u) {
            const u64 pos = off + j;
            if ((i64)pos < p.capacity) {
)QE";
    for (int i = 0; i < NO; i++) {
        const OutSpec &os = out.outs[i];
        const std::string ct = os.type == QE_BOOLEAN ? "unsigned char" : ctype(os.type);
        s << "                ((" << ct << " *)p.out[" << i << "])[pos] = ((const " << ct << " *)p.stage[" << i << "])[base + j];\n";
        if (os.nullable) s << "                p.outvalid[" << i << "][pos] = p.stagevalid[" << i << "][base + j];\n";
    }
    s << R"QE(            }
        }
    }
}
)QE";
}

void Emitter::filter_project() {
    filter_project_head();
    if (out.has_probe) conj_probe();
    ring_kernel();
    if (out.two_pass) two_pass_and_local();
}

void Emitter::gb_init_function(const char *comment) {
    s << comment << "__device__ __forceinline__ u64 qe_gb_init(int w) {\n    switch (w) {\n    case 0: return ~0ull;\n";
    for (int i = 0; i < NO; i++) {
        const int fn = in.agg_fns[i];
        if (fn == QE_AGG_MIN) s << "    case " << 2 + 2 * i << ": return 0x7fffffffffffffffull;\n";
        else if (fn == QE_AGG_MAX) s << "    case " << 2 + 2 * i << ": return 0x8000000000000000ull;\n";
    }
    s << "    default: return 0ull;\n    }\n}\n";
}
// ... 609 lines not shown
```

### queryengine_amd/csrc/qe_context.cpp

```cpp
#include <dlfcn.h>

#include <algorithm>
#include <atomic>
#include <cmath>
#include <cstdlib>
#include <sstream>

#include "qe_exec.h"
#include "qe_kernels.h"

namespace qe {

void fail(int32_t code, const std::string &msg) { throw Error{code, msg}; }

void hip_check(hipError_t e, const char *what, const char *file, int line) {
    if (e == hipSuccess) return;
    std::ostringstream s;
    s << what << " failed: " << hipGetErrorString(e) << " (" << (int)e << ") at " << file << ":" << line;
    fail(e == hipErrorOutOfMemory ? QE_ERR_OOM : QE_ERR_HIP, s.str());
}

uint64_t DictData::next_id() {
    static std::atomic<uint64_t> counter{0};
    return ++counter;
// ... 143 lines not shown
            return;
        }
        int ndev = 0;
        hipError_t e = hipGetDeviceCount(&ndev);
        if (e != hipSuccess || ndev == 0) {
            (void)hipGetLastError();
            fail(QE_ERR_HIP, std::string("no HIP device available: ") + hipGetErrorString(e) +
                                 " (libqe_hip has no CPU fallback)");
        }
        if (device < 0 || device >= ndev) fail(QE_ERR_INVALID_ARG, "device ordinal out of range");
        ctx = new qe_ctx();
        ctx->device = device;
        if (opts) {
            size_t n = std::min<size_t>(opts->struct_size, sizeof(qe_options));
            std::memcpy(&ctx->opts, opts, n);
        }
        ctx->opts.struct_size = sizeof(qe_options);
        QE_HIP(hipSetDevice(device));
        QE_HIP(hipStreamCreateWithFlags(&ctx->stream, hipStreamNonBlocking));
        QE_HIP(hipStreamCreateWithFlags(&ctx->copy_stream, hipStreamNonBlocking));
        QE_HIP(hipEventCreate(&ctx->ev0));
        QE_HIP(hipEventCreate(&ctx->ev1));
        QE_HIP(hipMalloc((void **)&ctx->d_ctrl, 256));
        QE_HIP(hipHostMalloc((void **)&ctx->h_ctrl, 256, hipHostMallocDefault));
        ctx->jit.reset(new Jit(ctx->opts.jit_cache_dir ? ctx->opts.jit_cache_dir : default_cache_dir()));
        ctx->opts.jit_cache_dir = nullptr;
    });
    if (st != QE_OK) {
        delete ctx;
        return st;
    }
    *out = ctx;
    return QE_OK;
}

void qe_ctx_destroy(qe_ctx *ctx) {
    if (!ctx) return;
    if (ctx->device < 0) {
        delete ctx;
        return;
    }
    (void)hipSetDevice(ctx->device);
    if (ctx->stream) (void)hipStreamSynchronize(ctx->stream);
    if (ctx->copy_stream) (void)hipStreamSynchronize(ctx->copy_stream);
    while (!ctx->host_results.empty()) qe_host_result_free(ctx, ctx->host_results.back());
    ctx->pinned.trim();
    qe_comm_destroy(ctx);
    ctx->plans.clear();
    ctx->jit.reset();
    ctx->pool.trim();
    if (ctx->d_ctrl) (void)hipFree(ctx->d_ctrl);
    if (ctx->h_ctrl) (void)hipHostFree(ctx->h_ctrl);
    if (ctx->ev0) (void)hipEventDestroy(ctx->ev0);
    if (ctx->ev1) (void)hipEventDestroy(ctx->ev1);
    if (ctx->stream) (void)hipStreamDestroy(ctx->stream);
    if (ctx->copy_stream) (void)hipStreamDestroy(ctx->copy_stream);
    delete ctx;
}

int32_t qe_ctx_set_exec_mode(qe_ctx *ctx, int32_t m) {
    if (!ctx || (m != QE_EXEC_FUSED && m != QE_EXEC_PER_NODE)) return QE_ERR_INVALID_ARG;
    ctx->opts.exec_mode = m;
    return QE_OK;
}
int32_t qe_ctx_set_cmp_semantics(qe_ctx *ctx, int32_t m) {
    if (!ctx || (m != QE_CMP_TOTAL_ORDER && m != QE_CMP_IEEE)) return QE_ERR_INVALID_ARG;
    ctx->opts.cmp_semantics = m;
    return QE_OK;
}
int32_t qe_ctx_kernel_time(qe_ctx *ctx, double *last_ms, double *total_ms, int64_t *launches) {
    if (!ctx) return QE_ERR_INVALID_ARG;
    if (last_ms) *last_ms = ctx->last_ms;
    if (total_ms) *total_ms = ctx->total_ms;
    if (launches) *launches = ctx->launches;
    return QE_OK;
}
int32_t qe_ctx_reset_kernel_time(qe_ctx *ctx) {
    if (!ctx) return QE_ERR_INVALID_ARG;
    ctx->last_ms = ctx->total_ms = 0.0;
    ctx->launches = 0;
    return QE_OK;
}
int32_t qe_ctx_last_form(const qe_ctx *ctx) { return ctx ? ctx->last_form : -1; }
int32_t qe_ctx_synchronize(qe_ctx *ctx) {
    if (!ctx) return QE_ERR_INVALID_ARG;
    return guarded(ctx, [&] { need_device(ctx); QE_HIP(hipStreamSynchronize(ctx->stream)); });
}
int32_t qe_ctx_trim(qe_ctx *ctx) {
    if (!ctx) return QE_ERR_INVALID_ARG;
    return guarded(ctx, [&] {
        need_device(ctx);
        QE_HIP(hipStreamSynchronize(ctx->stream));
        ctx->pool.trim();
        ctx->pinned.trim();
    });
}

int32_t qe_dict_create(qe_ctx *ctx, int32_t nentries, const char *const *utf8, qe_dict **out) {
    if (!ctx || !out || nentries < 0 || (nentries > 0 && !utf8)) return QE_ERR_INVALID_ARG;
    return guarded(ctx, [&] {
        auto d = std::make_shared<DictData>();
        d->entries.reserve(nentries);
        for (int32_t i = 0; i < nentries; i++) {
            if (!utf8[i]) fail(QE_ERR_INVALID_ARG, "null dictionary entry");
            d->entries.emplace_back(utf8[i]);
            d->index.emplace(d->entries.back(), i);
        }
        *out = new qe_dict{d};
    });
}
int32_t qe_dict_size(const qe_dict *dict) { return dict && dict->d ? (int32_t)dict->d->entries.size() : 0; }
const char *qe_dict_entry(const qe_dict *dict, int32_t code) {
    if (!dict || !dict->d || code < 0 || code >= (int32_t)dict->d->entries.size()) return nullptr;
    return dict->d->entries[code].c_str();
}
void qe_dict_free(qe_ctx *, qe_dict *dict) { delete dict; }

static void check_col_desc(const qe_col_desc &d, int64_t nrows) {
    if (d.type < QE_STRING || d.type > QE_INT32) fail(QE_ERR_INVALID_ARG, "bad column type");
    if (nrows > 0 && !d.data) fail(QE_ERR_INVALID_ARG, "null column data");
    if (d.type == QE_STRING && (!d.dict || !d.dict->d)) fail(QE_ERR_INVALID_ARG, "STRING column needs a dictionary");
}

int32_t qe_batch_create(qe_ctx *ctx, int64_t nrows, int32_t ncols, const qe_col_desc *cols, qe_batch **out) {
    if (!ctx || !out || nrows < 0 || ncols < 0 || (ncols > 0 && !cols)) return QE_ERR_INVALID_ARG;
    *out = nullptr;
    qe_batch *b = nullptr;
    int32_t st = guarded(ctx, [&] {
        need_device(ctx);
        b = new qe_batch();
        b->nrows = nrows;
        for (int32_t j = 0; j < ncols; j++) {
            check_col_desc(cols[j], nrows);
            Column c;
            c.type = cols[j].type;
            if (c.type == QE_STRING) c.dict = cols[j].dict->d;
            size_t nb = column_bytes(c.type, nrows);
            c.data = ctx->pool.alloc(nb);
            b->cols.push_back(c);
            if (nb) QE_HIP(hipMemcpyAsync(c.data, cols[j].data, nb, hipMemcpyHostToDevice, ctx->stream));
            if (cols[j].validity) {
                b->cols.back().validity = (uint64_t *)ctx->pool.alloc(bitmap_bytes(nrows));
                if (nrows > 0)
                    QE_HIP(hipMemcpyAsync(b->cols.back().validity, cols[j].validity, bitmap_bytes(nrows),
                                          hipMemcpyHostToDevice, ctx->stream));
            }
        }
        QE_HIP(hipStreamSynchronize(ctx->stream));
    });
    if (st != QE_OK) {
        free_batch(ctx, b);
        return st;
    }
    *out = b;
    return QE_OK;
}

int32_t qe_batch_wrap_device(qe_ctx *ctx, int64_t nrows, int32_t ncols, const qe_col_desc *cols, qe_batch **out) {
    if (!ctx || !out || nrows < 0 || ncols < 0 || (ncols > 0 && !cols)) return QE_ERR_INVALID_ARG;
    *out = nullptr;
    qe_batch *b = nullptr;
    int32_t st = guarded(ctx, [&] {
        b = new qe_batch();
        b->nrows = nrows;
        for (int32_t j = 0; j < ncols; j++) {
            check_col_desc(cols[j], nrows);
// ... 199 lines not shown
```

### queryengine_amd/csrc/qe_internal.h

```cpp
#pragma once

#include <hip/hip_runtime_api.h>

#include <cstdint>
#include <cstring>
#include <map>
#include <memory>
#include <string>
#include <unordered_map>
#include <vector>

#include "../../include/qe_hip.h"

namespace qe {

struct Error {
    int32_t code;
    std::string msg;
};
[[noreturn]] void fail(int32_t code, const std::string &msg);
void hip_check(hipError_t e, const char *what, const char *file, int line);
#define QE_HIP(x) ::qe::hip_check((x), #x, __FILE__, __LINE__)

enum NodeKind { N_COLUMN = 0, N_NUM = 1, N_BOOL = 2, N_STR = 3, N_FN = 4, N_CAST = 5, N_LIST = 6 };

struct Node {
    int kind = 0;
    int fn = -1;
    int type = -1;
    int col = -1;
    double num = 0.0;
    bool bval = false;
    std::string str;
    std::vector<double> list_num;
    std::vector<std::string> list_str;
    std::vector<char> list_bool;
    std::vector<int> ops;
};

struct Expr {
    std::vector<uint8_t> program;
    std::vector<Node> nodes;
    int root = -1;
    int max_stack = 0;
};

Expr decode_program(const uint8_t *program, size_t len);
int promote_type(int a, int b);
const char *type_name(int t);
const char *fn_name(int fn);

bool java_parse_double(const char *p, size_t n, double &out);
struct Field { size_t begin, end; bool quoted; };
bool next_record(const char *d, size_t n, size_t &pos, std::vector<Field> &fields, std::string &unq,
                 std::vector<std::pair<size_t, size_t>> &unq_span, bool &empty_line);

struct DictData {
    uint64_t id = next_id();
    static uint64_t next_id();
    std::vector<std::string> entries;
    std::unordered_map<std::string, int32_t> index;
    int32_t find(const std::string &s) const {
        auto it = index.find(s);
        return it == index.end() ? -1 : it->second;
    }
};

int utf16_compare(const std::string &a, const std::string &b);
std::vector<uint32_t> utf8_code_points(const std::string &s);
std::vector<std::vector<int32_t>> merged_ranks(const std::vector<const std::vector<std::string> *> &lists);

}

struct qe_dict {
    std::shared_ptr<qe::DictData> d;
};

namespace qe {

class Pool {
public:
    void *alloc(size_t bytes);
    void release(void *p);
    void trim();
    ~Pool() { trim_all(); }
    size_t bytes_in_use = 0, bytes_cached = 0;

private:
    void trim_all();
    std::multimap<size_t, void *> free_;
    std::unordered_map<void *, size_t> live_;
};

class PinnedPool {
public:
// ... 39 lines not shown

struct Column {
    int type = 0;
    void *data = nullptr;
    uint64_t *validity = nullptr;
    std::shared_ptr<DictData> dict;
    bool owned = true;
};

}

struct qe_batch {
    int64_t nrows = 0;
    bool schema_only = false;
    std::vector<qe::Column> cols;
    struct qe_result *view_of = nullptr;
};

struct qe_expr {
    qe::Expr e;
};

namespace qe {

struct OutColumn {
    int type = 0;
    bool nullable = false;
    void *data = nullptr;
    uint64_t *validity = nullptr;
    void *bytes_data = nullptr;
    uint8_t *bytes_valid = nullptr;
    std::shared_ptr<DictData> dict;
    qe_dict dict_handle;
    std::shared_ptr<void> hold_data, hold_valid;
};

}

struct qe_result {
    int64_t count = 0;
    int64_t capacity = 0;
    std::vector<qe::OutColumn> cols;
    int views = 0;
    bool free_pending = false;
};

namespace qe {

struct BoundColumn {
    int type;
    bool nullable;
    std::shared_ptr<DictData> dict;
};

struct OutSpec {
    int type;
    bool nullable;
    std::shared_ptr<DictData> dict;
};

inline int value_bytes(int type) { return type == QE_BOOLEAN ? 0 : (type == QE_DOUBLE || type == QE_INT64) ? 8 : 4; }
inline size_t output_row_bytes(const std::vector<OutSpec> &outs) {
    size_t n = 0;
    for (const OutSpec &o : outs) n += (o.type == QE_BOOLEAN ? 1 : value_bytes(o.type)) + (o.nullable ? 1 : 0);
    return n;
}

struct FusedGeometry {
    int threads = 256;
    int rows_per_lane = 2;
    int unroll = 8;
    int subs_per_chunk = 16;
    int nbuf = 2;
    int ring_entries = 256;
    int lookback_k = 1;
    int gate_period_log2 = 0;
    int gate_width_log2 = 0;
    int stagger = 0;
    int min_waves = 4;
    int prio_mode = 1;
    int resolve_at = 1;
    int sub_rows() const { return 64 * rows_per_lane * unroll; }
    int chunk_rows() const { return sub_rows() * subs_per_chunk; }
    int slot_rows() const { return chunk_rows() + 832; }
};

struct CodegenInput {
    const Expr *filter = nullptr;
    std::vector<const Expr *> projections;
    std::vector<int> agg_fns;
    std::vector<const Expr *> group_keys;
    std::vector<BoundColumn> schema;
    int cmp_semantics = QE_CMP_TOTAL_ORDER;
    FusedGeometry geo;
    int nontemporal = 1;
    int vec_stores = 0;
    int nt_stores = 1;
    int hp_shift = 0;
    int hp_lines = 1;
    int hp_parts = 0;
    std::vector<int> conj_order;
    int filter_load_stages = 0;
    int prefetch = 1;
    bool staged = true;
    bool dense = false;
    int debug_mask = 0;
};

struct CodegenOutput {
    std::string source;
    std::vector<OutSpec> outs;
    std::vector<int> used_cols;
    bool has_filter = false;
    bool two_pass = false;
    bool dense = false;
    bool has_probe = false;
    int nconj = 0;
    std::vector<std::vector<int>> conj_cols;
    std::vector<int> col_width;
    int fl_ring = 0;
    std::vector<std::vector<int32_t>> aux_tables;
    std::vector<OutSpec> keys;
    std::vector<int> key_domain;
    long long ngroups = 0;
    int table_words = 0;
    bool table_in_lds = false;
    bool hashed = false;
    int hash_words = 0;
    int table_copies = 1;
    std::vector<int> cnt_src;
    bool partitioned = false;
    int part_shift = 0;
    int part_groups = 0;
    int nparts = 0;
    std::vector<int> val_slot;
    int nvals = 0;
    bool hp = false;
    int hp_key_words = 0, hp_key_slot = 0, hp_shift = 11;
    int hp_line_recs = 0;
};

CodegenOutput generate_fused_source(const CodegenInput &in);
CodegenOutput analyze_fused_plan(const CodegenInput &in);

struct Kernel {
    hipModule_t module = nullptr;
    hipFunction_t fn = nullptr;
    int scratch = -1;
};

class Jit {
public:
    explicit Jit(std::string cache_dir) : cache_dir_(std::move(cache_dir)) {}
    ~Jit();
    Kernel get(const std::string &source, const char *entry, bool load = true);
    void reject(const std::string &source, int scratch);
    static std::vector<char> compile(const std::string &source);
    static std::string source_key(const std::string &source);
    int load_choice(const std::string &source, double *margin = nullptr) const;
    void store_choice(const std::string &source, int chosen, const std::string &note) const;
    static int scratch_bytes(const std::vector<char> &code);
    int compiles = 0, disk_hits = 0, mem_hits = 0, last_scratch = -1;

private:
    std::string cache_dir_;
    std::unordered_map<std::string, Kernel> loaded_;
};

struct Plan {
    CodegenOutput cg;
    Kernel kernel;
    FusedGeometry geo;
    bool aggregate = false;
    mutable std::vector<void *> aux_dev;
    ~Plan() { for (void *q : aux_dev) (void)hipFree(q); }
    mutable double last_selectivity = -1.0;
    mutable int64_t hash_capacity = 0;
    mutable int64_t id_capacity = 0;
    mutable bool use_ids = false;
    mutable int64_t known_keys = -1;
    mutable bool hp_failed = false;
    mutable bool ids_overflow = false;
    mutable std::vector<int> conj_order;
    mutable bool conj_decided = false;
    mutable bool local_overflowed = false;
    int est_regs = 0;
    bool explicit_geometry = false;
};

constexpr int kMaxCols = 16;
constexpr int kMaxOuts = 16;
struct FusedParams {
    const void *col[kMaxCols];
    const unsigned long long *colvalid[kMaxCols];
    void *out[kMaxOuts];
    unsigned char *outvalid[kMaxOuts];
    void *stage[kMaxOuts];
    unsigned char *stagevalid[kMaxOuts];
    long long nrows;
    long long capacity;
    unsigned long long *desc;
    unsigned long long *l1;
    unsigned long long *blk;
    unsigned int *ticket;
    unsigned long long *total;
    unsigned int *error;
    double *agg_partial;
    long long nchunks;
    long long stagger_chunks;
    long long stagger_rows;
    unsigned long long *trace;
    unsigned long long *stats;
};

}

struct qe_ctx {
    int device = 0;
    hipStream_t stream = nullptr;
    qe_options opts{};
    std::string last_error;
    qe::Pool pool;
    std::unique_ptr<qe::Jit> jit;
    std::map<std::string, std::shared_ptr<qe::Plan>> plans;
    struct GeoChoice {
        static constexpr int kCands = 3;
        int chosen = -1;
        int runs[kCands] = {0, 0, 0};
        float best_ms[kCands] = {1e30f, 1e30f, 1e30f};
        bool from_cache = false;
    };
    std::map<const qe::Plan *, GeoChoice> geo_choice;
    std::map<int64_t, std::shared_ptr<qe::DictData>> id_dicts;
    std::string source_scratch;
    hipEvent_t ev0 = nullptr, ev1 = nullptr;
    double last_ms = 0.0, total_ms = 0.0;
    int64_t launches = 0;
    unsigned int *d_ctrl = nullptr;
    unsigned long long *h_ctrl = nullptr;
    void *comm = nullptr;
    int comm_rank = -1, comm_nranks = 0;
    int last_form = -1;
    hipStream_t copy_stream = nullptr;
    qe::PinnedPool pinned;
    std::vector<struct qe_host_result *> host_results;
    qe_csv_device_stats csv_stats{};
    int64_t sort_stats[4] = {0, 0, 0, 0};
    int64_t join_stats[4] = {0, 0, 0, 0};
    int64_t window_stats[4] = {0, 0, 0, 0};
    int64_t ordered_stats[4] = {0, 0, 0, 0};
    int64_t set_stats[4] = {0, 0, 0, 0};
    int64_t asof_stats[4] = {0, 0, 0, 0};
};

struct qe_host_result {
    const qe_result *src = nullptr;
    int64_t count = 0;
    struct Col {
        int type = 0;
        bool nullable = false;
        void *data = nullptr;
        uint64_t *validity = nullptr;
        std::shared_ptr<qe::DictData> dict;
        qe_dict dict_handle;
    };
    std::vector<Col> cols;
    hipEvent_t done = nullptr;
    bool waited = false;
};

namespace qe {

class __attribute__((visibility("hidden"))) PoolScratch {
public:
    explicit PoolScratch(qe_ctx *ctx) : ctx_(ctx) {}
    PoolScratch(const PoolScratch &) = delete;
    PoolScratch &operator=(const PoolScratch &) = delete;
    ~PoolScratch() { for (void *p : bufs_) ctx_->pool.release(p); }
    void *alloc(size_t bytes) {
        bufs_.push_back(nullptr);
        return bufs_.back() = ctx_->pool.alloc(bytes);
    }

private:
    qe_ctx *ctx_;
    std::vector<void *> bufs_;
};

enum DebugBit : int {
    kDbgAblationMask = 255,
    kDbgWaitStats = 16,
    kDbgTrace = 32,
    kDbgScatterClocks = 64,
    kDbgGroupByGlobalAtomics = 256,
    kDbgForceTwoPass = 512,
    kDbgNeverTwoPass = 1024,
    kDbgNoLateMaterialisation = 2048,
    kDbgOneFilterLoadStage = 4096,
    kDbgNoGeometryChoice = 8192,
    kDbgForceDense = 16384,
    kDbgNeverDense = 32768,
    kDbgNoSelectivitySample = 65536,
    kDbgHashedGlobalAtomics = 131072,
    kDbgForceLocal = 262144,
    kDbgNeverLocal = 524288,
    kDbgWrittenConjunctOrder = 1048576,
    kDbgNoPrefetch = 2097152,
    kDbgAlwaysPrefetch = 4194304,
    kDbgForceHashPartitioned = 8388608,
    kDbgNeverHashPartitioned = 16777216,
    kDbgHpRecords = 33554432,
    kDbgGroupsOnDevice = 67108864,
};
inline bool debug_bit(const qe_ctx *ctx, DebugBit b) { return (ctx->opts.tuning[5] & b) != 0; }

}

std::vector<int64_t> qe_int_count_slices(qe_ctx *ctx, const qe_batch *batch, const qe_expr *filter, const qe_expr *const *projs, int32_t nproj,
                                         int64_t *slice_rows_io, int32_t nslices);
qe_result *qe_int_run_fused_slice(qe_ctx *ctx, const qe_batch *batch, int64_t row_begin, int64_t nrows, const qe_expr *filter,
                                  const qe_expr *const *projs, int32_t nproj);
```

### queryengine_amd/engine.py

```python
from __future__ import annotations

import ctypes as C
from typing import Any, Dict, List, Optional, Sequence

import numpy as np

from . import ast as A
from . import native as N
from .datatypes import DataType
from .program import serialize
from .table import Column, pack_bitmap, unpack_bitmap

_NP = {DataType.DOUBLE: np.float64, DataType.INT64: np.int64, DataType.INT32: np.int32, DataType.STRING: np.int32}


def window_frame_fn(f: Sequence) -> tuple:
    f = tuple(int(v) for v in f)
    if len(f) <= 3:
        fn = f[0] if f else -1
        running = N.WIN_SUM <= fn <= N.WIN_AVG
        return (f + (0, 0, 0))[:3] + ((N.FRAME_UNBOUNDED, 0) if running else (0, 0))
    return (f + (0,))[:5]


def MEDIAN(column: int) -> tuple:
    return (N.OSA_PERCENTILE_CONT, int(column), 0.5)


def ordered_agg(f: Sequence) -> tuple:
    f = tuple(f)
    if not 2 <= len(f) <= 3:
        raise ValueError("an ordered-set aggregate is (fn, column) or (fn, column, fraction)")
    return (int(f[0]), int(f[1]), float(f[2]) if len(f) == 3 else 0.0)


class Context:

    def __init__(self, device: Optional[int] = 0, exec_mode: int = N.EXEC_FUSED, cmp_semantics: int = N.CMP_TOTAL_ORDER,
                 profile: bool = False, result_capacity_rows: int = 0, jit_cache_dir: Optional[str] = None,
                 tuning: Sequence[int] = ()):
        self._lib = N.lib()
        opts = N.Options()
        opts.struct_size = C.sizeof(N.Options)
        opts.exec_mode = exec_mode
        opts.cmp_semantics = cmp_semantics
        opts.profile = 1 if profile else 0
        opts.result_capacity_rows = result_capacity_rows
        opts.jit_cache_dir = jit_cache_dir.encode() if jit_cache_dir else None
        for i, t in enumerate(tuning):
            opts.tuning[i] = int(t)
        h = C.c_void_p()
        st = self._lib.qe_ctx_create(N.DEVICE_NONE if device is None else device, C.byref(opts), C.byref(h))
        N.check(None, st)
        self.handle = h
        self.device = device
        self._dicts: Dict[tuple, "Dictionary"] = {}

    def close(self) -> None:
        if getattr(self, "handle", None):
            self._dicts.clear()
            self._lib.qe_ctx_destroy(self.handle)
            self.handle = None

    def __enter__(self):
        return self

    def __exit__(self, *exc):
        self.close()

    def __del__(self):
        try:
            self.close()
        except Exception:
            pass

    def set_exec_mode(self, mode: int) -> None:
        N.check(self.handle, self._lib.qe_ctx_set_exec_mode(self.handle, mode))

    def set_cmp_semantics(self, mode: int) -> None:
        N.check(self.handle, self._lib.qe_ctx_set_cmp_semantics(self.handle, mode))

    def kernel_time(self):
        last, total, n = C.c_double(), C.c_double(), C.c_int64()
        N.check(self.handle, self._lib.qe_ctx_kernel_time(self.handle, C.byref(last), C.byref(total), C.byref(n)))
        return last.value, total.value, n.value

    def reset_kernel_time(self) -> None:
        N.check(self.handle, self._lib.qe_ctx_reset_kernel_time(self.handle))

    @property
    def last_form(self) -> int:
        return int(self._lib.qe_ctx_last_form(self.handle))

    def synchronize(self) -> None:
        N.check(self.handle, self._lib.qe_ctx_synchronize(self.handle))

    def trim(self) -> None:
        N.check(self.handle, self._lib.qe_ctx_trim(self.handle))

    def stream_read_bandwidth(self, nbytes: int = 1 << 30, reps: int = 5) -> float:
        out = C.c_double()
        N.check(self.handle, self._lib.qe_stream_read_bandwidth(self.handle, nbytes, reps, C.byref(out)))
        return out.value

    def stream_read_write_time(self, nbytes: int, write_every: int, reps: int = 5):
        ms, wb = C.c_double(), C.c_double()
        N.check(self.handle, self._lib.qe_stream_read_write_time(self.handle, nbytes, write_every, reps, C.byref(ms), C.byref(wb)))
        return ms.value, wb.value

    def comm_unique_id(self) -> bytes:
        buf = C.create_string_buffer(N.COMM_ID_BYTES)
        N.check(self.handle, self._lib.qe_comm_unique_id(self.handle, buf))
        return buf.raw

    def comm_init(self, nranks: int, rank: int, unique_id: bytes) -> None:
        assert len(unique_id) == N.COMM_ID_BYTES
        buf = C.create_string_buffer(unique_id, N.COMM_ID_BYTES)
        N.check(self.handle, self._lib.qe_comm_init(self.handle, nranks, rank, buf))

    @property
    def comm_rank(self) -> int:
        return int(self._lib.qe_comm_rank(self.handle))

    @property
    def comm_nranks(self) -> int:
        return int(self._lib.qe_comm_nranks(self.handle))

    def comm_destroy(self) -> None:
        self._lib.qe_comm_destroy(self.handle)

    def gather(self, result: "Result", root: int = 0) -> Optional["Result"]:
        h = C.c_void_p()
        N.check(self.handle, self._lib.qe_gather(self.handle, result.handle, root, C.byref(h)))
        return Result(self, h) if h.value else None

    def filter_project_gather(self, batch: "DeviceBatch", filter: Optional["CompiledExpression"], projections: Sequence["CompiledExpression"],
                              root: int = 0, nslices: int = 0) -> Optional["Result"]:
        h = C.c_void_p()
        N.check(self.handle, self._lib.qe_filter_project_gather(self.handle, batch.handle, filter.handle if filter else None,
                                                                _expr_array(projections), len(projections), root, nslices, C.byref(h)))
        return Result(self, h) if h.value else None

    def allgather_host(self, payload: bytes) -> List[bytes]:
        n = self.comm_nranks
        recv = C.create_string_buffer(len(payload) * n)
        N.check(self.handle, self._lib.qe_comm_allgather_host(self.handle, payload, len(payload), recv))
        return [recv.raw[i * len(payload):(i + 1) * len(payload)] for i in range(n)]

    def order_by(self, result: "Result", column: int) -> "Result":
        h = C.c_void_p()
        N.check(self.handle, self._lib.qe_result_order_by(self.handle, result.handle, column, C.byref(h)))
        return Result(self, h)

    def order_by_keys(self, result: "Result", keys: Sequence, limit: Optional[int] = None) -> "Result":
        keys = list(keys)
        arr = (N.SortKey * max(1, len(keys)))(*[N.SortKey(int(c), 1 if d else 0) for c, d in keys])
        h = C.c_void_p()
        N.check(self.handle, self._lib.qe_result_order_by_keys(self.handle, result.handle, arr, len(keys),
                                                               -1 if limit is None else int(limit), C.byref(h)))
        return Result(self, h)

    def last_sort_stats(self) -> dict:
        out = (C.c_int64 * 4)()
        N.check(self.handle, self._lib.qe_ctx_last_sort_stats(self.handle, out))
        return {"path": "select" if out[0] == 1 else "sort", "sorted_rows": int(out[1]), "radix_passes": int(out[2]),
                "select_passes": int(out[3])}

    def join_build(self, side, key_cols: Sequence[int]) -> "JoinTable":
        return JoinTable(self, side, key_cols)

    def last_join_stats(self) -> List[int]:
        out = (C.c_int64 * 4)()
        N.check(self.handle, self._lib.qe_ctx_last_join_stats(self.handle, out))
        return [int(v) for v in out]

# ... 460 lines not shown
```

### queryengine_amd/native.py

```python
from __future__ import annotations

import ctypes as C
import importlib.util
import os
import sys
import subprocess
from typing import List, Optional, Sequence

import numpy as np

from .datatypes import DataType

_HERE = os.path.dirname(os.path.abspath(__file__))
CSRC = os.path.join(_HERE, "csrc")
LIB_PATH = os.path.join(CSRC, "libqe_hip.so")

OK = 0
ERR_NAMES = {1: "INVALID_ARG", 2: "PROGRAM", 3: "HIP", 4: "OOM", 5: "UNSUPPORTED", 6: "INTERNAL", 7: "COMM"}
DEVICE_NONE = -1
EXEC_FUSED, EXEC_PER_NODE = 0, 1
CMP_TOTAL_ORDER, CMP_IEEE = 0, 1
GEN_I64_MOD, GEN_I32_MOD, GEN_F64_UNIT, GEN_F64_MOD, GEN_F64_STEP, GEN_F64_PRICE, GEN_DICT_MOD, GEN_I64_ROWID = range(8)
AGG_MIN, AGG_MAX, AGG_SUM, AGG_COUNT, AGG_AVG = range(5)
COMM_ID_BYTES = 128
FORM_RING, FORM_TWO_PASS, FORM_DENSE, FORM_PER_NODE, FORM_NO_FILTER, FORM_LOCAL = range(6)
FORM_GROUPBY_DENSE, FORM_GROUPBY_HASHED, FORM_GROUPBY_HASH_PARTITIONED = 8, 9, 10
JOIN_INNER, JOIN_LEFT, JOIN_SEMI, JOIN_ANTI = range(4)
WIN_ROW_NUMBER, WIN_RANK, WIN_DENSE_RANK, WIN_SUM, WIN_COUNT, WIN_MIN, WIN_MAX, WIN_AVG, WIN_LAG, WIN_LEAD = range(10)
WIN_FIRST_VALUE, WIN_LAST_VALUE = 10, 11
FRAME_UNBOUNDED = -1
WIN_TILE_ROWS, WIN_TRIP_TILES = 2048, 1024
OSA_COUNT_DISTINCT, OSA_PERCENTILE_CONT, OSA_PERCENTILE_DISC, OSA_MODE = range(4)
OSA_BLOCKS = 1024
OSA_WORD_BLOCKS = 128
SET_UNION, SET_INTERSECT, SET_EXCEPT = range(3)
SETOP_BLOCKS = 2048
ASOF_BACKWARD, ASOF_FORWARD = range(2)
ASOF_BLOCKS = 2048


class QeError(RuntimeError):
    def __init__(self, code: int, msg: str):
        super().__init__(f"[QE_ERR_{ERR_NAMES.get(code, code)}] {msg}")
        self.code = code


class Options(C.Structure):
    _fields_ = [("struct_size", C.c_uint32), ("exec_mode", C.c_int32), ("cmp_semantics", C.c_int32),
                ("profile", C.c_int32), ("result_capacity_rows", C.c_int64), ("jit_cache_dir", C.c_char_p),
                ("tuning", C.c_int32 * 8)]


class ColDesc(C.Structure):
    _fields_ = [("type", C.c_int32), ("reserved", C.c_int32), ("data", C.c_void_p), ("validity", C.c_void_p),
                ("dict", C.c_void_p)]


class GenSpec(C.Structure):
    _fields_ = [("kind", C.c_int32), ("col_id", C.c_int32), ("modulus", C.c_uint64), ("offset", C.c_int64),
                ("step", C.c_double), ("aux_col_id", C.c_int32), ("null_pct", C.c_int32), ("dict", C.c_void_p)]


class ColView(C.Structure):
    _fields_ = [("type", C.c_int32), ("nullable", C.c_int32), ("data", C.c_void_p), ("validity", C.c_void_p),
                ("count", C.c_int64), ("dict", C.c_void_p)]


class CsvDeviceStats(C.Structure):
    _fields_ = [("text_bytes", C.c_int64), ("nrows", C.c_int64), ("host_patched_fields", C.c_int64),
                ("host_fallback", C.c_int32), ("reserved", C.c_int32), ("h2d_ms", C.c_double), ("kernel_ms", C.c_double)]


class SortKey(C.Structure):
    _fields_ = [("column", C.c_int32), ("descending", C.c_int32)]


class JoinInput(C.Structure):
    _fields_ = [("result", C.c_void_p), ("batch", C.c_void_p)]


class WindowFn(C.Structure):
    _fields_ = [("fn", C.c_int32), ("column", C.c_int32), ("offset", C.c_int64)]


class WindowFrameFn(C.Structure):
    _fields_ = [("fn", C.c_int32), ("column", C.c_int32), ("offset", C.c_int64), ("preceding", C.c_int64), ("following", C.c_int64)]


class OrderedAgg(C.Structure):
    _fields_ = [("fn", C.c_int32), ("column", C.c_int32), ("fraction", C.c_double)]


_P = C.c_void_p
SYMBOLS = [
    ("qe_abi_version", C.c_int32, []),
    ("qe_last_error", C.c_char_p, [_P]),
    ("qe_ctx_create", C.c_int32, [C.c_int32, C.POINTER(Options), C.POINTER(_P)]),
    ("qe_ctx_destroy", None, [_P]),
    ("qe_ctx_set_exec_mode", C.c_int32, [_P, C.c_int32]),
    ("qe_ctx_set_cmp_semantics", C.c_int32, [_P, C.c_int32]),
    ("qe_ctx_kernel_time", C.c_int32, [_P, C.POINTER(C.c_double), C.POINTER(C.c_double), C.POINTER(C.c_int64)]),
    ("qe_ctx_reset_kernel_time", C.c_int32, [_P]),
    ("qe_ctx_last_form", C.c_int32, [_P]),
    ("qe_ctx_synchronize", C.c_int32, [_P]),
    ("qe_ctx_trim", C.c_int32, [_P]),
    ("qe_dict_create", C.c_int32, [_P, C.c_int32, C.POINTER(C.c_char_p), C.POINTER(_P)]),
    ("qe_dict_size", C.c_int32, [_P]),
    ("qe_dict_entry", C.c_char_p, [_P, C.c_int32]),
    ("qe_dict_free", None, [_P, _P]),
    ("qe_batch_create", C.c_int32, [_P, C.c_int64, C.c_int32, C.POINTER(ColDesc), C.POINTER(_P)]),
    ("qe_batch_wrap_device", C.c_int32, [_P, C.c_int64, C.c_int32, C.POINTER(ColDesc), C.POINTER(_P)]),
    ("qe_batch_describe", C.c_int32, [_P, C.c_int64, C.c_int32, C.POINTER(ColDesc), C.POINTER(_P)]),
    ("qe_batch_generate", C.c_int32, [_P, C.c_uint64, C.c_int64, C.c_int64, C.c_int32, C.POINTER(GenSpec), C.POINTER(_P)]),
    ("qe_batch_nrows", C.c_int64, [_P]),
    ("qe_batch_ncols", C.c_int32, [_P]),
    ("qe_batch_column_type", C.c_int32, [_P, C.c_int32]),
    ("qe_batch_column_to_host", C.c_int32, [_P, _P, C.c_int32, C.c_int64, C.c_int64, _P, _P]),
    ("qe_batch_free", None, [_P, _P]),
    ("qe_csv_parse", C.c_int32, [_P, C.c_char_p, C.c_size_t, C.c_int32, C.POINTER(C.c_char_p), C.POINTER(C.c_int32), C.POINTER(_P)]),
    ("qe_csv_parse_file", C.c_int32, [_P, C.c_char_p, C.c_int32, C.POINTER(C.c_char_p), C.POINTER(C.c_int32), C.POINTER(_P)]),
    ("qe_csv_nrows", C.c_int64, [_P]),
    ("qe_csv_ncols", C.c_int32, [_P]),
    ("qe_csv_column", C.c_int32, [_P, C.c_int32, C.POINTER(ColDesc)]),
    ("qe_csv_pin", C.c_int32, [_P, _P, C.POINTER(_P)]),
    ("qe_csv_free", None, [_P, _P]),
    ("qe_csv_parse_device", C.c_int32, [_P, C.c_char_p, C.c_size_t, C.c_int32, C.POINTER(C.c_char_p), C.POINTER(C.c_int32), C.POINTER(_P)]),
    ("qe_csv_parse_file_device", C.c_int32, [_P, C.c_char_p, C.c_int32, C.POINTER(C.c_char_p), C.POINTER(C.c_int32), C.POINTER(_P)]),
    ("qe_csv_device_last_stats", C.c_int32, [_P, C.POINTER(CsvDeviceStats)]),
    ("qe_batch_column_nullable", C.c_int32, [_P, C.c_int32]),
    ("qe_batch_column_dict", C.c_int32, [_P, C.c_int32, C.POINTER(_P)]),
    ("qe_expr_compile", C.c_int32, [_P, C.c_char_p, C.c_size_t, C.POINTER(_P)]),
    ("qe_expr_result_type", C.c_int32, [_P]),
    ("qe_expr_free", None, [_P, _P]),
    ("qe_filter_project", C.c_int32, [_P, _P, _P, C.POINTER(_P), C.c_int32, C.POINTER(_P)]),
    ("qe_filter_project_prepare", C.c_int32, [_P, _P, _P, C.POINTER(_P), C.c_int32]),
    ("qe_filter_aggregate", C.c_int32, [_P, _P, _P, C.POINTER(_P), C.POINTER(C.c_int32), C.c_int32,
                                        C.POINTER(C.c_double), C.POINTER(C.c_uint8), C.POINTER(C.c_int64)]),
    ("qe_filter_groupby", C.c_int32, [_P, _P, _P, C.POINTER(_P), C.c_int32, C.POINTER(_P), C.POINTER(C.c_int32), C.c_int32, C.POINTER(_P)]),
    ("qe_filter_groupby_prepare", C.c_int32, [_P, _P, _P, C.POINTER(_P), C.c_int32, C.POINTER(_P), C.POINTER(C.c_int32), C.c_int32]),
    ("qe_filter_aggregate_prepare", C.c_int32, [_P, _P, _P, C.POINTER(_P), C.POINTER(C.c_int32), C.c_int32]),
    ("qe_result_count", C.c_int64, [_P]),
    ("qe_result_ncols", C.c_int32, [_P]),
    ("qe_result_column", C.c_int32, [_P, C.c_int32, C.POINTER(ColView)]),
    ("qe_result_column_to_host", C.c_int32, [_P, _P, C.c_int32, _P, _P]),
    ("qe_result_free", None, [_P, _P]),
    ("qe_result_to_host", C.c_int32, [_P, _P, C.POINTER(_P)]),
    ("qe_host_result_wait", C.c_int32, [_P, _P]),
    ("qe_host_result_count", C.c_int64, [_P]),
    ("qe_host_result_ncols", C.c_int32, [_P]),
    ("qe_host_result_column", C.c_int32, [_P, C.c_int32, C.POINTER(ColView)]),
    ("qe_host_result_free", None, [_P, _P]),
    ("qe_result_concat", C.c_int32, [_P, C.POINTER(_P), C.c_int32, C.POINTER(_P)]),
    ("qe_result_order_by", C.c_int32, [_P, _P, C.c_int32, C.POINTER(_P)]),
    ("qe_result_order_by_keys", C.c_int32, [_P, _P, _P, C.c_int32, C.c_int64, C.POINTER(_P)]),
    ("qe_ctx_last_sort_stats", C.c_int32, [_P, C.POINTER(C.c_int64)]),
    ("qe_join_build", C.c_int32, [_P, C.POINTER(JoinInput), C.POINTER(C.c_int32), C.c_int32, C.POINTER(_P)]),
    ("qe_join_table_rows", C.c_int64, [_P]),
    ("qe_join_table_free", None, [_P, _P]),
    ("qe_join_probe", C.c_int32, [_P, _P, C.POINTER(JoinInput), C.POINTER(C.c_int32), C.c_int32, C.c_int32,
                                  C.POINTER(C.c_int32), C.c_int32, C.POINTER(C.c_int32), C.c_int32, C.POINTER(_P)]),
    ("qe_ctx_last_join_stats", C.c_int32, [_P, C.POINTER(C.c_int64)]),
    ("qe_result_window", C.c_int32, [_P, _P, C.POINTER(C.c_int32), C.c_int32, _P, C.c_int32, C.POINTER(WindowFn), C.c_int32, C.POINTER(_P)]),
    ("qe_result_window_frames", C.c_int32, [_P, _P, C.POINTER(C.c_int32), C.c_int32, _P, C.c_int32, C.POINTER(WindowFrameFn), C.c_int32, C.POINTER(_P)]),
    ("qe_ctx_last_window_stats", C.c_int32, [_P, C.POINTER(C.c_int64)]),
    ("qe_result_group_ordered", C.c_int32, [_P, _P, C.POINTER(C.c_int32), C.c_int32, C.POINTER(OrderedAgg), C.c_int32, C.POINTER(_P)]),
    ("qe_ctx_last_ordered_stats", C.c_int32, [_P, C.POINTER(C.c_int64)]),
    ("qe_result_set_op", C.c_int32, [_P, _P, _P, C.c_int32, C.c_int32, C.POINTER(_P)]),
    ("qe_ctx_last_set_stats", C.c_int32, [_P, C.POINTER(C.c_int64)]),
    ("qe_result_asof_join", C.c_int32, [_P, _P, _P, C.POINTER(C.c_int32), C.POINTER(C.c_int32), C.c_int32, C.c_int32, C.c_int32,
                                        C.c_int32, C.c_int32, C.c_int32, C.POINTER(C.c_int32), C.c_int32, C.POINTER(C.c_int32), C.c_int32,
                                        C.POINTER(_P)]),
    ("qe_ctx_last_asof_stats", C.c_int32, [_P, C.POINTER(C.c_int64)]),
    ("qe_batch_from_result", C.c_int32, [_P, _P, C.POINTER(_P)]),
    ("qe_comm_unique_id", C.c_int32, [_P, _P]),
    ("qe_comm_init", C.c_int32, [_P, C.c_int32, C.c_int32, _P]),
    ("qe_comm_rank", C.c_int32, [_P]),
    ("qe_comm_nranks", C.c_int32, [_P]),
    ("qe_comm_destroy", None, [_P]),
    ("qe_gather", C.c_int32, [_P, _P, C.c_int32, C.POINTER(_P)]),
    ("qe_filter_project_gather", C.c_int32, [_P, _P, _P, C.POINTER(_P), C.c_int32, C.c_int32, C.c_int32, C.POINTER(_P)]),
    ("qe_comm_allgather_host", C.c_int32, [_P, _P, C.c_size_t, _P]),
    ("qe_filter_project_source", C.c_int32, [_P, _P, _P, C.POINTER(_P), C.c_int32, C.POINTER(C.c_char_p)]),
    ("qe_filter_project_geometry", C.c_int32, [_P, _P, _P, C.POINTER(_P), C.c_int32, C.POINTER(C.c_int32), C.POINTER(C.c_int32)]),
    ("qe_filter_project_conjunct_order", C.c_int32, [_P, _P, _P, C.POINTER(_P), C.c_int32, C.POINTER(C.c_int32), C.c_int32, C.POINTER(C.c_int32)]),
    ("qe_stream_read_bandwidth", C.c_int32, [_P, C.c_int64, C.c_int32, C.POINTER(C.c_double)]),
    ("qe_stream_read_write_time", C.c_int32, [_P, C.c_int64, C.c_int32, C.c_int32, C.POINTER(C.c_double), C.POINTER(C.c_double)]),
# ... 58 lines not shown
```

Baseline: 319.4 billion.

## Replace per-chunk LDS ring buffers with one circular queue per wave

The per-wave fixed set of LDS buffers (one per queued chunk) becomes a single circular queue of NBUF*RING entries. Each queued chunk occupies a variable span that starts where its predecessor's ended, and up to four chunks may be queued at once. Rows spill to staging only when a load group's kept rows do not fit the free entries, which is meant to cut spills and forced waits at mixed selectivity. In exchange, slot indexing now uses a modulo on a capacity that may not be a power of two, staging grows to four slots per wave, and occupancy queries are cached per plan.

```diff
diff --git a/include/qe_hip.h b/include/qe_hip.h
--- a/include/qe_hip.h
+++ b/include/qe_hip.h
@@ -281,6 +281,7 @@
         QE_FORM_GROUPBY_DENSE = 8, QE_FORM_GROUPBY_HASHED = 9,
        QE_FORM_GROUPBY_HASH_PARTITIONED = 10  };
 int32_t qe_ctx_last_form(const qe_ctx *ctx);
+int32_t qe_ctx_last_ring_stats(const qe_ctx *ctx, int64_t out[4]);
 int32_t qe_stream_read_bandwidth(qe_ctx *ctx, int64_t nbytes, int32_t reps, double *out_gbps);
 
 int32_t qe_stream_read_write_time(qe_ctx *ctx, int64_t nbytes, int32_t write_every, int32_t reps, double *out_ms,
diff --git a/queryengine_amd/csrc/qe_api.cpp b/queryengine_amd/csrc/qe_api.cpp
--- a/queryengine_amd/csrc/qe_api.cpp
+++ b/queryengine_amd/csrc/qe_api.cpp
@@ -245,11 +245,11 @@
         if (ctx->opts.tuning[7] / 100 == 0) in.geo.nbuf = 2;
         if (ctx->opts.tuning[0] == 0) {
             const size_t limit = 96 * 1024;
-            while (in.geo.threads > 64 && (size_t)(in.geo.threads / 64) * in.geo.nbuf * in.geo.ring_entries * rowbytes > limit)
+            while (in.geo.threads > 64 && in.geo.queue_lds_bytes(rowbytes) > limit)
                 in.geo.threads /= 2;
         }
-        if ((size_t)(in.geo.threads / 64) * in.geo.nbuf * in.geo.ring_entries * rowbytes > 156 * 1024)
-            fail(QE_ERR_UNSUPPORTED, "projection list too wide for the fused kernel's LDS buffers (" + std::to_string(rowbytes) +
+        if (in.geo.queue_lds_bytes(rowbytes) > 156 * 1024)
+            fail(QE_ERR_UNSUPPORTED, "projection list too wide for the fused kernel's LDS queue (" + std::to_string(rowbytes) +
                                          " bytes per output row); use QE_EXEC_PER_NODE");
     }
 }
@@ -351,13 +351,16 @@
 
 int blocks_per_cu(const qe_ctx *ctx, const Plan &plan) {
     if (ctx->opts.tuning[3] % 100 > 0) return ctx->opts.tuning[3] % 100;
-    int nb = 0;
-    hipError_t e = hipModuleOccupancyMaxActiveBlocksPerMultiprocessor(&nb, plan.kernel.fn, plan.geo.threads, 0);
-    if (e != hipSuccess) {
-        (void)hipGetLastError();
-        nb = 2;
-    }
-    return std::max(1, std::min(nb, 8));
+    if (plan.occupancy_blocks == 0) {
+        int nb = 0;
+        hipError_t e = hipModuleOccupancyMaxActiveBlocksPerMultiprocessor(&nb, plan.kernel.fn, plan.geo.threads, 0);
+        if (e != hipSuccess) {
+            (void)hipGetLastError();
+            nb = 2;
+        }
+        plan.occupancy_blocks = std::max(1, std::min(nb, 8));
+    }
+    return plan.occupancy_blocks;
 }
 
 std::vector<int> choose_conjunct_order(qe_ctx *ctx, const qe_batch *batch, const Plan &plan) {
@@ -412,11 +415,12 @@
 
 
 
+constexpr size_t kCtrlBytes = 104;
 template <typename Launch>
 const unsigned int *with_ctrl_block(qe_ctx *ctx, Launch &&launch) {
-    QE_HIP(hipMemsetAsync(ctx->d_ctrl, 0, 96, ctx->stream));
+    QE_HIP(hipMemsetAsync(ctx->d_ctrl, 0, kCtrlBytes, ctx->stream));
     launch();
-    QE_HIP(hipMemcpyAsync(ctx->h_ctrl, ctx->d_ctrl, 96, hipMemcpyDeviceToHost, ctx->stream));
+    QE_HIP(hipMemcpyAsync(ctx->h_ctrl, ctx->d_ctrl, kCtrlBytes, hipMemcpyDeviceToHost, ctx->stream));
     QE_HIP(hipStreamSynchronize(ctx->stream));
     collect_time(ctx);
     return (const unsigned int *)ctx->h_ctrl;
@@ -733,15 +737,16 @@
     if (nchunks >= (1ll << 31)) fail(QE_ERR_UNSUPPORTED, "batch too large for 32-bit chunk tickets");
     const int grid = (int)std::min<int64_t>((nchunks + waves - 1) / waves, max_grid);
     static const bool dbg_grid = std::getenv("QE_DEBUG_GRID") != nullptr;
-    if (dbg_grid) std::fprintf(stderr, "[qe] ring kernel: grid %d x %d threads (%d blocks per CU), unroll %d, %d sub-tiles per chunk, ring %d, min_waves %d\n",
-                               grid, plan.geo.threads, blocks_per_cu(ctx, plan), plan.geo.unroll, plan.geo.subs_per_chunk, plan.geo.ring_entries, plan.geo.min_waves);
+    if (dbg_grid) std::fprintf(stderr, "[qe] ring kernel: grid %d x %d threads (%d blocks per CU), unroll %d, %d sub-tiles per chunk, queue %d x %d = %d entries, %d chunks queued at most, min_waves %d\n",
+                               grid, plan.geo.threads, blocks_per_cu(ctx, plan), plan.geo.unroll, plan.geo.subs_per_chunk, plan.geo.nbuf, plan.geo.ring_entries,
+                               plan.geo.queue_entries(), kRingQueueMaxChunks, plan.geo.min_waves);
     PoolScratch scratch(ctx);
     const int64_t nblocks = (nchunks + 63) / 64;
     const size_t desc_words = (size_t)nchunks + 2 * (size_t)nblocks;
     unsigned long long *desc = (unsigned long long *)scratch.alloc(desc_words * 8);
     FusedParams p = r.p;
     if (plan.cg.has_filter) {
-        const size_t slots = (size_t)grid * waves * plan.geo.nbuf;
+        const size_t slots = (size_t)grid * waves * kRingQueueMaxChunks;
         alloc_staging(r, scratch, p, slots * (size_t)plan.geo.slot_rows());
     }
     p.capacity = r.cap;
@@ -765,7 +770,12 @@
     if (debug_bit(ctx, kDbgWaitStats))
         std::fprintf(stderr, "[qe stats] chunks %llu failed_tries %llu forced_waits %llu blocking_spins %llu\n", ctx->h_ctrl[11],
                      ctx->h_ctrl[8], ctx->h_ctrl[10], ctx->h_ctrl[9]);
+    if (hc[1] == 6) fail(QE_ERR_INTERNAL, "fused kernel: the LDS queue's accounting found no row to spill");
     if (hc[1] != 0) fail(QE_ERR_INTERNAL, "fused kernel: look-back spin limit reached (tile descriptor never published)");
+    ctx->ring_stats[0] = nchunks;
+    ctx->ring_stats[1] = (int64_t)ctx->h_ctrl[1];
+    ctx->ring_stats[2] = (int64_t)ctx->h_ctrl[12];
+    ctx->ring_stats[3] = plan.cg.has_filter ? plan.geo.queue_entries() : 0;
     return (int64_t)ctx->h_ctrl[1];
 }
 
diff --git a/queryengine_amd/csrc/qe_codegen.cpp b/queryengine_amd/csrc/qe_codegen.cpp
--- a/queryengine_amd/csrc/qe_codegen.cpp
+++ b/queryengine_amd/csrc/qe_codegen.cpp
@@ -1557,9 +1557,12 @@
 
 void Emitter::ring_defs() {
     const FusedGeometry &geo = in.geo;
-    s << "\n#define QE_NBUF " << geo.nbuf << "u\n#define QE_RING " << geo.ring_entries << "   // LDS entries per wave, buffer and output column (power of two)\n";
+    s << "\n#define QE_NBUF " << geo.nbuf << "u\n#define QE_RING " << geo.ring_entries << "\n";
+    s << "#define QE_QCAP (QE_NBUF * QE_RING)   // LDS entries per wave and output column: ONE circular queue\n";
+    s << "#define QE_QMAX " << kRingQueueMaxChunks << "u   // chunks a wave may have queued at a time\n";
     s << "#define QE_FL_RING " << out.fl_ring << "\n";
-    s << "struct QeRing {\n";
+    s << "#define QE_RQ_FN __device__ __forceinline__\n" << qe_ring_queue_text << "\n";
+    s << "struct QeRing {\n    u32 first;   // entry of the chunk's row 0 (the local form: 0)\n";
     for (int i = 0; i < NO; i++) {
         const OutSpec &os = out.outs[i];
         s << "    " << (os.type == QE_BOOLEAN ? "unsigned char" : ctype(os.type)) << " *r" << i << ";\n";
@@ -1931,12 +1934,17 @@
         return;
     }
     // rows are ordered (u, lane, r) inside the sub-tile: lane offsets from ballots; the ring belongs to this wave only
+    (void)flushed;
 #pragma unroll
     for (int u = 0; u < QE_U; ++u) {
         const u64 b0 = __ballot(keep[u][0]);
         const u64 b1 = __ballot(keep[u][1]);
+        const u32 cnt = (u32)__popcll(b0) + (u32)__popcll(b1);
+        // single-pass form: the wave's queue spills (run / flushed are the caller's) only if these cnt rows do not fit;
+        // the local form (MODE 3) flags the overflow at the end of its chunk instead
+        if constexpr (MODE == 0) after_loads.room(cnt);
         const u32 off = run + qe_mbcnt(b0) + qe_mbcnt(b1);
-        run += (u32)__popcll(b0) + (u32)__popcll(b1);
+        run += cnt;
 #pragma unroll
         for (int r = 0; r < 2; ++r) {
             if (keep[u][r] && (QE_DEBUG_MASK & 2)) {   // ablation build: keep the outputs (and their loads) alive
@@ -1944,7 +1952,8 @@
     for (int i = 0; i < NO; i++) s << "                asm volatile(\"\" :: \"v\"(o" << i << "[u][r]));\n";
     s << R"QE(            }
             if (keep[u][r] && !(QE_DEBUG_MASK & 2)) {
-                const u32 slot = (off + (r == 1 && keep[u][0] ? 1u : 0u)) & ((MODE == 3 ? QE_FL_RING : QE_RING) - 1);
+                const u32 j = off + (r == 1 && keep[u][0] ? 1u : 0u);
+                const u32 slot = MODE == 3 ? (j & (QE_FL_RING - 1)) : qe_rq_entry(QE_QCAP, ring.first, j);
 )QE";
     for (int i = 0; i < NO; i++) {
         const OutSpec &os = out.outs[i];
@@ -1952,17 +1961,7 @@
         else s << "                ring.r" << i << "[slot] = o" << i << "[u][r];\n";
         if (os.nullable) s << "                ring.rv" << i << "[slot] = ok" << i << "[u][r] ? 1 : 0;\n";
     }
-    s << "            }\n        }\n";
-    s << "        while (MODE != 3 && run - flushed >= QE_RING - 128u) {   // only when the ring would overflow (high selectivity); the local form (MODE 3) flags the overflow at the end of its chunk instead\n";
-    s << "            const u32 src = (flushed + lane) & (QE_RING - 1);\n";
-    s << "            const u64 dst = stage_base + flushed + lane;\n            if (!(QE_DEBUG_MASK & 8)) {\n";
-    for (int i = 0; i < NO; i++) {
-        const OutSpec &os = out.outs[i];
-        const std::string ct = os.type == QE_BOOLEAN ? "unsigned char" : ctype(os.type);
-        s << "            QE_SPILL_ST((" << ct << " *)p.stage[" << i << "] + dst, ring.r" << i << "[src]);\n";
-        if (os.nullable) s << "            QE_SPILL_ST(p.stagevalid[" << i << "] + dst, ring.rv" << i << "[src]);\n";
-    }
-    s << "            }\n            flushed += 64u;\n        }\n    }\n}\n";
+    s << "            }\n        }\n    }\n}\n";
 }
 
 void Emitter::passthrough_tail() {
@@ -2271,6 +2270,13 @@
 )QE";
     if (has_filter) {
         s << R"QE(
+// What the single-pass kernel hands qe_sub: the work it issues under a sub-tile's loads, and the queue's spill rule.
+template <typename Under, typename Room> struct QeSubHooks {
+    Under &under;
+    Room &make_room;
+    __device__ __forceinline__ void operator()() const { under(); }
+    __device__ __forceinline__ void room(const u32 cnt) const { make_room(cnt); }
+};
 // The exclusive prefix of a streamed chunk is known: tell the successors at once.
 __device__ __forceinline__ void qe_publish_prefix(const QeParams &p, const i64 pchunk, const u32 prun, const u64 excl, const int lane) {
     if (lane == 0 && pchunk > 0)
@@ -2287,8 +2293,8 @@
 }
 // Finish a streamed chunk whose exclusive prefix is known: publish the inclusive prefix, then move the
 // staged rows to their final, globally ordered position (coalesced both ways, 4 blocks in flight).
-// Rows [0, pflushed) of the chunk were spilled to the wave's staging slot (only when the LDS buffer
-// overflowed); rows [pflushed, prun) are still in the LDS buffer `ring`.
+// Rows [0, pflushed) of the chunk were spilled to its staging slot (only when the wave's LDS queue
+// overflowed); rows [pflushed, prun) are still in the queue, row j at entry (ring.first + j) mod QE_QCAP.
 __device__ __forceinline__ void qe_finish(const QeParams &p, const i64 pchunk, const u32 prun, const u32 pflushed, const u64 pbase,
                                           const u64 excl, const int lane, const QeRing &ring, const bool publish = true) {
     if (publish) qe_publish_prefix(p, pchunk, prun, excl, lane);
@@ -2306,8 +2312,8 @@
         for (int i = 0; i < NO; i++) {
             const OutSpec &os = out.outs[i];
             const std::string ct = os.type == QE_BOOLEAN ? "unsigned char" : ctype(os.type);
-            s << "                QE_ST((" << ct << " *)p.out[" << i << "] + pos, ring.r" << i << "[jv & (QE_RING - 1)]);\n";
-            if (os.nullable) s << "                QE_ST(p.outvalid[" << i << "] + pos, ring.rv" << i << "[jv & (QE_RING - 1)]);\n";
+            s << "                QE_ST((" << ct << " *)p.out[" << i << "] + pos, ring.r" << i << "[qe_rq_entry(QE_QCAP, ring.first, jv)]);\n";
+            if (os.nullable) s << "                QE_ST(p.outvalid[" << i << "] + pos, ring.rv" << i << "[qe_rq_entry(QE_QCAP, ring.first, jv)]);\n";
         }
         s << R"QE(            }
             jv++;
@@ -2320,7 +2326,7 @@
         for (int i = 0; i < NO; i++) {
             const OutSpec &os = out.outs[i];
             const std::string ct = os.type == QE_BOOLEAN ? "unsigned char" : ctype(os.type);
-            const std::string a = "ring.r" + std::to_string(i) + "[j & (QE_RING - 1)]", b = "ring.r" + std::to_string(i) + "[(j + 1u) & (QE_RING - 1)]";
+            const std::string a = "ring.r" + std::to_string(i) + "[qe_rq_entry(QE_QCAP, ring.first, j)]", b = "ring.r" + std::to_string(i) + "[qe_rq_entry(QE_QCAP, ring.first, j + 1u)]";
             if (os.type == QE_DOUBLE || os.type == QE_INT64) {
                 const std::string vt = os.type == QE_DOUBLE ? "qe_f64x2" : "qe_i64x2";
                 s << "                if (two) { " << vt << " v2; v2.x = " << a << "; v2.y = " << b << "; QE_ST((" << vt << " *)((" << ct << " *)p.out[" << i
@@ -2330,8 +2336,8 @@
                   << "] + pos + 1, " << b << ");\n";
             }
             if (os.nullable)
-                s << "                QE_ST(p.outvalid[" << i << "] + pos, ring.rv" << i << "[j & (QE_RING - 1)]);\n                if (two) QE_ST(p.outvalid[" << i
-                  << "] + pos + 1, ring.rv" << i << "[(j + 1u) & (QE_RING - 1)]);\n";
+                s << "                QE_ST(p.outvalid[" << i << "] + pos, ring.rv" << i << "[qe_rq_entry(QE_QCAP, ring.first, j)]);\n                if (two) QE_ST(p.outvalid[" << i
+                  << "] + pos + 1, ring.rv" << i << "[qe_rq_entry(QE_QCAP, ring.first, j + 1u)]);\n";
         }
         s << R"QE(            }
         }
@@ -2343,8 +2349,8 @@
         for (int i = 0; i < NO; i++) {
             const OutSpec &os = out.outs[i];
             const std::string ct = os.type == QE_BOOLEAN ? "unsigned char" : ctype(os.type);
-            s << "                QE_ST((" << ct << " *)p.out[" << i << "] + pos, ring.r" << i << "[j & (QE_RING - 1)]);\n";
-            if (os.nullable) s << "                QE_ST(p.outvalid[" << i << "] + pos, ring.rv" << i << "[j & (QE_RING - 1)]);\n";
+            s << "                QE_ST((" << ct << " *)p.out[" << i << "] + pos, ring.r" << i << "[qe_rq_entry(QE_QCAP, ring.first, j)]);\n";
+            if (os.nullable) s << "                QE_ST(p.outvalid[" << i << "] + pos, ring.rv" << i << "[qe_rq_entry(QE_QCAP, ring.first, j)]);\n";
         }
         s << R"QE(            }
         }
@@ -2382,12 +2388,14 @@
     }
     s << R"QE(
 // Every WAVE is an independent worker: it draws a chunk of consecutive rows with one ticket, streams it
-// sub-tile by sub-tile and (with a Filter) compacts the kept rows into one of its QE_NBUF private LDS
-// buffers, then publishes the chunk's count.  Chunk ids are monotone in start order, so a look-back only
-// ever waits on chunks that are already running.  Streamed chunks queue up in the wave's FIFO of LDS
-// buffers; the OLDEST one is resolved (look-back + move) NON-BLOCKINGLY at sub-tile boundaries while the
-// wave keeps streaming newer chunks; the wave waits only when every buffer is taken.  At low selectivity
-// the rows never leave LDS before they are written to their final position.  No barrier.
+// sub-tile by sub-tile and (with a Filter) compacts the kept rows into its private circular LDS queue of
+// QE_QCAP entries, then publishes the chunk's count.  Chunk ids are monotone in start order, so a look-back
+// only ever waits on chunks that are already running.  Streamed chunks stay queued (up to QE_QMAX of them,
+// each a span of the queue that starts where its predecessor's ended); the OLDEST one is resolved
+// (look-back + move) NON-BLOCKINGLY at sub-tile boundaries while the wave keeps streaming newer chunks; the
+// wave waits only when QE_QMAX chunks are queued.  Rows are spilled to a staging slot only when a load
+// group's kept rows do not fit the free entries, oldest rows first (qe_ring_queue.h): unless the queue
+// overflows, the rows never leave LDS before they are written to their final position.  No barrier.
 extern "C" __global__ void __launch_bounds__(QE_THREADS, QE_MIN_WAVES) qe_fused(const QeParams p) {
     const int lane = threadIdx.x & 63;
     const int wv = __builtin_amdgcn_readfirstlane(threadIdx.x >> 6);
@@ -2398,10 +2406,11 @@
         for (int i = 0; i < NO; i++) {
             const OutSpec &os = out.outs[i];
             const std::string ct = os.type == QE_BOOLEAN ? "unsigned char" : ctype(os.type);
-            s << "    __shared__ " << ct << " s_r" << i << "[QE_WAVES][QE_NBUF * QE_RING];\n";
-            if (os.nullable) s << "    __shared__ unsigned char s_rv" << i << "[QE_WAVES][QE_NBUF * QE_RING];\n";
-        }
-        s << "    __shared__ u32 s_meta[QE_WAVES][QE_NBUF][4];   // per queued chunk: id, kept rows, rows spilled to staging\n";
+            s << "    __shared__ " << ct << " s_r" << i << "[QE_WAVES][QE_QCAP];\n    ring.r" << i << " = s_r" << i << "[wv]; pring.r" << i << " = s_r" << i << "[wv];\n";
+            if (os.nullable)
+                s << "    __shared__ unsigned char s_rv" << i << "[QE_WAVES][QE_QCAP];\n    ring.rv" << i << " = s_rv" << i << "[wv]; pring.rv" << i << " = s_rv" << i << "[wv];\n";
+        }
+        s << "    __shared__ u32 s_meta[QE_WAVES][QE_QMAX][4];   // per queued chunk: id, first entry, kept rows, rows spilled to staging\n";
     } else {
         for (int i = 0; i < NO; i++) {
             s << "    ring.r" << i << " = nullptr; pring.r" << i << " = nullptr;\n";
@@ -2409,8 +2418,12 @@
         }
     }
     s << R"QE(    (void)wv;
-    u32 cur = 0;                 // LDS buffer being filled
-    u32 npend = 0;               // streamed chunks queued in buffers cur-npend .. cur-1 (mod QE_NBUF), oldest first
+    ring.first = 0; pring.first = 0;
+    u32 cur = 0;                 // position (staging slot, s_meta row) of the chunk being filled
+    u32 npend = 0;               // streamed chunks queued at positions cur-npend .. cur-1 (mod QE_QMAX), oldest first
+    u32 qstart = 0;              // queue entry of the filling chunk's row 0: where the previous chunk's span ended
+    u32 qlive = 0;               // rows of the queued chunks that are in LDS (not spilled)
+    u64 st_spilled = 0;          // rows this wave spilled to staging
     i64 hchunk = 0;              // the oldest queued chunk (head of the FIFO) ...
     u32 hrun = 0, hflushed = 0;  // ... its kept rows and how many of them were spilled to its staging slot
     bool hvalid = false;         // head fields + look-back state are loaded
@@ -2429,19 +2442,18 @@
 )QE";
     if (has_filter) {
         s << R"QE(    auto load_head = [&]() {
-        const u32 h = (cur + QE_NBUF - npend) % QE_NBUF;
+        const u32 h = (cur + QE_QMAX - npend) % QE_QMAX;
         hchunk = (i64)s_meta[wv][h][0];
-        hrun = s_meta[wv][h][1];
-        hflushed = s_meta[wv][h][2];
+        pring.first = __builtin_amdgcn_readfirstlane(s_meta[wv][h][1]);
+        hrun = __builtin_amdgcn_readfirstlane(s_meta[wv][h][2]);
+        hflushed = __builtin_amdgcn_readfirstlane(s_meta[wv][h][3]);
         qe_lb_init(lb, hchunk);
         hvalid = true;
-)QE";
-        for (int i = 0; i < NO; i++) {
-            s << "        pring.r" << i << " = s_r" << i << "[wv] + h * QE_RING;\n";
-            if (out.outs[i].nullable) s << "        pring.rv" << i << " = s_rv" << i << "[wv] + h * QE_RING;\n";
-        }
-        s << R"QE(    };
-    auto head_base = [&]() { return ((u64)wslot * QE_NBUF + (cur + QE_NBUF - npend) % QE_NBUF) * QE_SLOT_ROWS; };
+    };
+    auto slot_base = [&](const u32 pos) { return ((u64)wslot * QE_QMAX + pos) * QE_SLOT_ROWS; };   // one staging slot per (wave, queue position)
+    auto head_base = [&]() { return slot_base((cur + QE_QMAX - npend) % QE_QMAX); };
+    // The head left the queue (moved to its final position): its LDS rows are free again.
+    auto pop_head = [&]() { qlive -= hrun - hflushed; npend--; hvalid = false; hres = false; };
 )QE";
     }
     s << R"QE(    for (;;) {
@@ -2456,22 +2468,64 @@
         const i64 chunk = (i64)(u32)__builtin_amdgcn_readfirstlane(t);
         const bool have = chunk < p.nchunks;
         if ((QE_DEBUG_MASK & 32) && have && lane == 0) p.trace[chunk * 4 + 0] = __builtin_amdgcn_s_memrealtime();
-        const u64 stage_base = ((u64)wslot * QE_NBUF + cur) * QE_SLOT_ROWS;
+        const u64 stage_base = ((u64)wslot * QE_QMAX + cur) * QE_SLOT_ROWS;
         u32 run = 0, flushed = 0;
-)QE";
-    if (has_filter) {
-        for (int i = 0; i < NO; i++) {
-            s << "        ring.r" << i << " = s_r" << i << "[wv] + cur * QE_RING;\n";
-            if (out.outs[i].nullable) s << "        ring.rv" << i << " = s_rv" << i << "[wv] + cur * QE_RING;\n";
-        }
-    }
-    s << R"QE(        if (have) {
+        ring.first = qstart;
+        if (have) {
             i64 row0, rend;
             qe_chunk_range(p, chunk, row0, rend);
             i64 sub = row0;
             u32 si = 0;
-            // issued right after each sub-tile's loads, so that its stores / polls run under them
-            auto hook = [&]() {
+)QE";
+    if (has_filter) {
+        s << R"QE(            // Exact: rows are spilled only if the `cnt` kept rows of this load group do not fit the free entries of the
+            // queue, and then the OLDEST rows in LDS leave first, 64 at a time: those of the oldest queued chunk that still
+            // has any, of the filling chunk when no queued one has.  Either way rows [0, spilled) of a chunk are in its
+            // staging slot and the rest in LDS, which is what qe_finish expects.  Never waits.
+            auto make_room = [&](const u32 cnt) {
+                while (qe_rq_must_spill(QE_QCAP, qlive + (run - flushed), cnt)) {
+                    u32 pos = cur, first = qstart, from = flushed, n = qe_rq_block_rows(run - flushed);
+                    bool queued = false;
+                    for (u32 k = npend; k > 0 && qlive > 0; --k) {
+                        const u32 q = (cur + QE_QMAX - k) % QE_QMAX;
+                        const u32 krun = __builtin_amdgcn_readfirstlane(s_meta[wv][q][2]);
+                        const u32 kfl = __builtin_amdgcn_readfirstlane(s_meta[wv][q][3]);
+                        if (krun != kfl) {
+                            pos = q; first = __builtin_amdgcn_readfirstlane(s_meta[wv][q][1]); from = kfl;
+                            n = qe_rq_block_rows(krun - kfl);
+                            queued = true;
+                            if (k == npend && hvalid) hflushed = kfl + n;   // the head's fields are held in registers too
+                            break;
+                        }
+                    }
+                    if (n == 0u) {   // bounded like the spins: the accounting says "full" and nothing is in LDS -- report, never loop
+                        if (lane == 0) *p.error = 6u;
+                        break;
+                    }
+                    if ((u32)lane < n && !(QE_DEBUG_MASK & 8)) {
+                        const u32 src = qe_rq_entry(QE_QCAP, first, from + lane);
+                        const u64 dst = slot_base(pos) + from + lane;
+)QE";
+        for (int i = 0; i < NO; i++) {
+            const OutSpec &os = out.outs[i];
+            const std::string ct = os.type == QE_BOOLEAN ? "unsigned char" : ctype(os.type);
+            s << "                        QE_SPILL_ST((" << ct << " *)p.stage[" << i << "] + dst, ring.r" << i << "[src]);\n";
+            if (os.nullable) s << "                        QE_SPILL_ST(p.stagevalid[" << i << "] + dst, ring.rv" << i << "[src]);\n";
+        }
+        s << R"QE(                    }
+                    if (queued) {
+                        if (lane == 0) s_meta[wv][pos][3] = from + n;
+                        qlive -= n;
+                    } else {
+                        flushed += n;
+                    }
+                    st_spilled += n;
+                }
+            };
+)QE";
+    }
+    s << R"QE(            // issued right after each sub-tile's loads, so that its stores / polls run under them
+            auto under_loads = [&]() {
 )QE";
     if (has_filter)
         s << "                if (pub_owed) { qe_publish_complete(p, pub_chunk, pub_run, pub_old, lane); pub_owed = false; }\n";
@@ -2488,9 +2542,11 @@
              "                    // resolved: move the rows now, or (gated build) in the next window / before the buffer is needed\n"
              "                    if (hres && (si + 2 >= QE_SUBS_PER_CHUNK || qe_gate_open())) {\n"
              "                        qe_finish(p, hchunk, hrun, hflushed, head_base(), hexcl, lane, pring, false);\n"
-             "                        npend--; hvalid = false; hres = false;\n                    }\n                }\n";
-    s << R"QE(            };
-            if (QE_PRIO_MODE == 2) qe_rotate_priority(nchunk_done);
+             "                        pop_head();\n                    }\n                }\n";
+    s << "            };\n";
+    if (has_filter) s << "            const QeSubHooks<decltype(under_loads), decltype(make_room)> hook{under_loads, make_room};\n";
+    else s << "            auto &hook = under_loads;\n";
+    s << R"QE(            if (QE_PRIO_MODE == 2) qe_rotate_priority(nchunk_done);
             QePf pf;
 #if QE_PREFETCH
             if (sub + QE_SUB_ROWS <= rend) qe_s0_load(p, sub, lane, pf);   // the chunk's first sub-tile; every later one is prefetched by its predecessor
@@ -2519,14 +2575,17 @@
                 p.trace[chunk * 4 + 3] = ((u64)wslot << 40) | ((u64)(__builtin_amdgcn_s_getreg((20 << 0) | (0 << 6) | (3 << 11)) & 0xf) << 32) |
                                          (u64)(u32)__builtin_amdgcn_s_getreg((4 << 0) | (0 << 6) | (31 << 11));
             }
-            if (lane == 0) { s_meta[wv][cur][0] = (u32)chunk; s_meta[wv][cur][1] = run; s_meta[wv][cur][2] = flushed; }
+            // queue it: its span ends where the next chunk's starts
+            if (lane == 0) { s_meta[wv][cur][0] = (u32)chunk; s_meta[wv][cur][1] = qstart; s_meta[wv][cur][2] = run; s_meta[wv][cur][3] = flushed; }
+            qlive += run - flushed;
+            qstart = qe_rq_entry(QE_QCAP, qstart, run);
             npend++;
-            cur = (cur + 1u) % QE_NBUF;
+            cur = (cur + 1u) % QE_QMAX;
             st_chunks++;
         }
-        if (pub_owed && (npend == QE_NBUF || !have)) { qe_publish_complete(p, pub_chunk, pub_run, pub_old, lane); pub_owed = false; }
-        // every buffer is taken (or nothing is left to stream): now the wave may wait for the oldest chunk
-        while (npend == QE_NBUF || (!have && npend > 0)) {
+        if (pub_owed && (npend == QE_QMAX || !have)) { qe_publish_complete(p, pub_chunk, pub_run, pub_old, lane); pub_owed = false; }
+        // QE_QMAX chunks are queued (or nothing is left to stream): now the wave may wait for the oldest chunk
+        while (npend == QE_QMAX || (!have && npend > 0)) {
             if (!hvalid) load_head();
             if (QE_DEBUG_MASK & 16) {
                 st_forced++;
@@ -2536,16 +2595,18 @@
             }
             const u64 excl = hres ? hexcl : ((QE_DEBUG_MASK & 1) ? 0ull : qe_lookback_wait(p, hchunk, lb, lane));
             qe_finish(p, hchunk, hrun, hflushed, head_base(), excl, lane, pring, !hres);
-            npend--; hvalid = false; hres = false;
+            pop_head();
         }
         if (!have) break;
 )QE";
     } else {
         s << "            if (lane == 0 && chunk == p.nchunks - 1) *p.total = (u64)p.nrows;\n        }\n";
-        s << "        (void)npend; (void)hchunk; (void)hrun; (void)hflushed; (void)hvalid; (void)hres; (void)hexcl; (void)cur; (void)pring; (void)run; (void)flushed; (void)lb;\n";
+        s << "        (void)npend; (void)hchunk; (void)hrun; (void)hflushed; (void)hvalid; (void)hres; (void)hexcl; (void)cur; (void)pring; (void)run; (void)flushed; (void)lb; (void)qstart; (void)qlive; (void)st_spilled;\n";
         s << "        if (!have) break;\n";
     }
     s << "    }\n";
+    if (has_filter)
+        s << "    if (st_spilled != 0 && lane == 0) atomicAdd(p.stats + 4, st_spilled);\n";
     if (has_filter)
         s << "    if ((QE_DEBUG_MASK & 16) && lane == 0) { atomicAdd(p.stats + 0, st_fail); atomicAdd(p.stats + 1, st_spin); "
              "atomicAdd(p.stats + 2, st_forced); atomicAdd(p.stats + 3, st_chunks); }\n";
@@ -2616,7 +2677,8 @@
         if (os.nullable) s << "    __shared__ unsigned char s_lv" << i << "[QE_WAVES][QE_FL_RING];\n    ring.rv" << i << " = s_lv" << i << "[wv];\n";
     }
     if (NO == 0) s << "    ring.unused = 0;\n";
-    s << R"QE(    u32 nsub_done = 0;
+    s << R"QE(    ring.first = 0;
+    u32 nsub_done = 0;
     QePf pf;
     bool pf_have = false;   // `pf` holds the stage-0 columns of the next full sub-tile this wave works on (also across its chunks)
     (void)pf_have;
diff --git a/queryengine_amd/csrc/qe_context.cpp b/queryengine_amd/csrc/qe_context.cpp
--- a/queryengine_amd/csrc/qe_context.cpp
+++ b/queryengine_amd/csrc/qe_context.cpp
@@ -249,6 +249,11 @@
     return QE_OK;
 }
 int32_t qe_ctx_last_form(const qe_ctx *ctx) { return ctx ? ctx->last_form : -1; }
+int32_t qe_ctx_last_ring_stats(const qe_ctx *ctx, int64_t out[4]) {
+    if (!ctx || !out) return QE_ERR_INVALID_ARG;
+    for (int i = 0; i < 4; i++) out[i] = ctx->ring_stats[i];
+    return QE_OK;
+}
 int32_t qe_ctx_synchronize(qe_ctx *ctx) {
     if (!ctx) return QE_ERR_INVALID_ARG;
     return guarded(ctx, [&] { need_device(ctx); QE_HIP(hipStreamSynchronize(ctx->stream)); });
diff --git a/queryengine_amd/csrc/qe_internal.h b/queryengine_amd/csrc/qe_internal.h
--- a/queryengine_amd/csrc/qe_internal.h
+++ b/queryengine_amd/csrc/qe_internal.h
@@ -11,6 +11,7 @@
 #include <vector>
 
 #include "../../include/qe_hip.h"
+#include "qe_ring_queue.h"
 
 namespace qe {
 
@@ -216,6 +217,8 @@
     int resolve_at = 1;
     int sub_rows() const { return 64 * rows_per_lane * unroll; }
     int chunk_rows() const { return sub_rows() * subs_per_chunk; }
+    int queue_entries() const { return nbuf * ring_entries; }
+    size_t queue_lds_bytes(size_t rowbytes) const { return (size_t)(threads / 64) * (size_t)queue_entries() * rowbytes; }
     int slot_rows() const { return chunk_rows() + 832; }
 };
 
@@ -317,6 +320,7 @@
     mutable bool ids_overflow = false;
     mutable std::vector<int> conj_order;
     mutable bool conj_decided = false;
+    mutable int occupancy_blocks = 0;
     mutable bool local_overflowed = false;
     int est_regs = 0;
     bool explicit_geometry = false;
@@ -384,6 +388,7 @@
     int64_t window_stats[4] = {0, 0, 0, 0};
     int64_t ordered_stats[4] = {0, 0, 0, 0};
     int64_t set_stats[4] = {0, 0, 0, 0};
+    int64_t ring_stats[4] = {0, 0, 0, 0};
     int64_t asof_stats[4] = {0, 0, 0, 0};
 };
 
diff --git a/queryengine_amd/csrc/qe_ring_queue.h b/queryengine_amd/csrc/qe_ring_queue.h
--- /dev/null
+++ b/queryengine_amd/csrc/qe_ring_queue.h
@@ -0,0 +1,33 @@
+#pragma once
+
+#define QE_RING_QUEUE_BODY                                                                                               \
+                    \
+    QE_RQ_FN unsigned qe_rq_free(const unsigned cap, const unsigned live) { return cap - live; }                        \
+                               \
+    QE_RQ_FN bool qe_rq_must_spill(const unsigned cap, const unsigned live, const unsigned need) {                      \
+        return need > qe_rq_free(cap, live);                                                                            \
+    }                                                                                                                   \
+                                    \
+    QE_RQ_FN unsigned qe_rq_block_rows(const unsigned chunk_live) { return chunk_live < 64u ? chunk_live : 64u; }       \
+                                       \
+    QE_RQ_FN unsigned qe_rq_blocks(const unsigned cap, const unsigned live, const unsigned need,                        \
+                                   const unsigned chunk_live) {                                                         \
+        if (!qe_rq_must_spill(cap, live, need)) return 0u;                                                              \
+        const unsigned missing = need - qe_rq_free(cap, live);                                                          \
+        const unsigned take = missing < chunk_live ? missing : chunk_live;                                              \
+        return (take + 63u) / 64u;                                                                                      \
+    }                                                                                                                   \
+                                                         \
+    QE_RQ_FN unsigned qe_rq_entry(const unsigned cap, const unsigned first, const unsigned j) {                         \
+        return (first + j) % cap;                                                                                       \
+    }
+
+#define QE_RQ_STR2(...) #__VA_ARGS__
+#define QE_RQ_STR(x) QE_RQ_STR2(x)
+static const char qe_ring_queue_text[] = QE_RQ_STR(QE_RING_QUEUE_BODY);
+
+#define QE_RQ_FN static inline
+QE_RING_QUEUE_BODY
+#undef QE_RQ_FN
+
+constexpr int kRingQueueMaxChunks = 4;
diff --git a/queryengine_amd/engine.py b/queryengine_amd/engine.py
--- a/queryengine_amd/engine.py
+++ b/queryengine_amd/engine.py
@@ -91,6 +91,11 @@
     @property
     def last_form(self) -> int:
         return int(self._lib.qe_ctx_last_form(self.handle))
+
+    def last_ring_stats(self) -> dict:
+        out = (C.c_int64 * 4)()
+        N.check(self.handle, self._lib.qe_ctx_last_ring_stats(self.handle, out))
+        return {"chunks": int(out[0]), "kept": int(out[1]), "spilled": int(out[2]), "queue_entries": int(out[3])}
 
     def synchronize(self) -> None:
         N.check(self.handle, self._lib.qe_ctx_synchronize(self.handle))
diff --git a/queryengine_amd/native.py b/queryengine_amd/native.py
--- a/queryengine_amd/native.py
+++ b/queryengine_amd/native.py
@@ -102,6 +102,7 @@
     ("qe_ctx_kernel_time", C.c_int32, [_P, C.POINTER(C.c_double), C.POINTER(C.c_double), C.POINTER(C.c_int64)]),
     ("qe_ctx_reset_kernel_time", C.c_int32, [_P]),
     ("qe_ctx_last_form", C.c_int32, [_P]),
+    ("qe_ctx_last_ring_stats", C.c_int32, [_P, C.POINTER(C.c_int64)]),
     ("qe_ctx_synchronize", C.c_int32, [_P]),
     ("qe_ctx_trim", C.c_int32, [_P]),
     ("qe_dict_create", C.c_int32, [_P, C.c_int32, C.POINTER(C.c_char_p), C.POINTER(_P)]),
```

New measurement: 317.3 billion. No clear change (-0.7%).
